# microsoft/MaskFlownet

Hardware: NVIDIA H100
Metric: image-pairs/sec (MaskFlownet-S forward, 1024x448) (higher is better)
Workload: dtype f32

## Files before the change

### include/maskflow_b200.h

```cpp
#ifndef MASKFLOW_B200_H_
#define MASKFLOW_B200_H_

#ifdef __cplusplus
extern "C" {
#endif

#define MFN_VERSION 100

#if defined(__GNUC__)
#define MFN_API __attribute__((visibility("default")))
#else
#define MFN_API
#endif

#define MFN_OK 0
#define MFN_ERR_INVALID_ARG (-1)
#define MFN_ERR_UNSUPPORTED (-2)
#define MFN_ERR_ALIGNMENT (-3)

#define MFN_CORR_AUTO 0
#define MFN_CORR_GENERIC 1
#define MFN_CORR_SIMT 2
#define MFN_CORR_MMA_BF16X3 3

#define MFN_BORDER_MXNET15 0
#define MFN_BORDER_ZERO_CORNER 1

MFN_API int mfn_version(void);
MFN_API const char* mfn_last_error(void);
MFN_API const char* mfn_last_kernel(void);
MFN_API unsigned long long mfn_launch_count(void);
MFN_API int mfn_set_tuning(const char* key, int value);

MFN_API int mfn_correlation_forward(const float* data1, const float* data2, float* out, int N, int C, int H,
                            int W, int pad_size, int kernel_size, int max_displacement, int stride1,
                            int stride2, int is_multiply, long long out_batch_stride,
                            float leaky_slope, int algo, void* stream);

MFN_API int mfn_correlation_backward(const float* grad_out, const float* out, const float* data1,
                             const float* data2, float* grad1, float* grad2, int N, int C, int H,
                             int W, int max_displacement, long long out_batch_stride,
                             float leaky_slope, void* stream);

MFN_API int mfn_deformable_conv_forward(const float* data, const float* offset, const float* weight,
                                const float* bias, float* out, int N, int C, int H, int W, int F,
                                int kernel_h, int kernel_w, int stride_h, int stride_w, int dilate_h,
                                int dilate_w, int pad_h, int pad_w, int num_group,
                                int num_deformable_group, int border_mode, void* stream);

MFN_API int mfn_deformable_conv_backward(const float* grad_out, const float* data, const float* offset,
                                 const float* weight, float* grad_data, float* grad_offset,
                                 float* grad_weight, float* grad_bias, int N, int C, int H, int W,
                                 int F, int border_mode, void* stream);

MFN_API int mfn_warp_mask_forward(const float* x, const float* flow_coarse, const float* mask_coarse,
                          const float* weight, const float* bias, const float* tradeoff, float* out,
                          float* flow_up_out, float* mask_up_out, float* conv_out, int N, int C,
                          int H, int W, int F, int upsample_factor, float flow_scale,
                          float level_stride, float leaky_slope, int border_mode, void* stream);

MFN_API int mfn_warp_mask_forward_tc(const float* x, const float* flow_coarse, const float* mask_coarse,
                                     const void* packed_weight, const float* bias, const float* tradeoff, float* out,
                                     float* flow_up_out, float* mask_up_out, float* conv_out, int N, int C, int H, int W,
                                     int F, int upsample_factor, float flow_scale, float level_stride, float leaky_slope,
                                     int border_mode, void* stream);

MFN_API long long mfn_warp_resample_workspace_bytes(int N, int F, int H, int W);
MFN_API int mfn_warp_mask_forward_resample(const float* x, const float* flow_coarse, const float* mask_coarse,
                                           const float* weight, const void* packed_weight, const float* bias,
                                           const float* tradeoff, void* workspace, float* out, float* flow_up_out,
                                           float* mask_up_out, int N, int C, int H, int W, int F, int upsample_factor,
                                           float flow_scale, float level_stride, float leaky_slope, int border_mode,
                                           void* stream);

MFN_API int mfn_warp_mask_backward(const float* grad_out, const float* out, const float* conv_out,
                           const float* x, const float* flow_up, const float* mask_up,
                           const float* weight, float* grad_x, float* grad_flow_up,
                           float* grad_mask_up, float* grad_weight, float* grad_bias,
                           float* grad_tradeoff, float* grad_conv_ws, int N, int C, int H, int W,
                           int F, float flow_scale, float level_stride, float leaky_slope,
                           int border_mode, void* stream);

MFN_API int mfn_upsample_forward(const float* in, float* out, int planes, int H, int W, int factor,
                         float scale, void* stream);
MFN_API int mfn_upsample_backward(const float* grad_out, float* grad_in, int planes, int H, int W, int factor,
                          float scale, void* stream);

MFN_API int mfn_grid_generator_warp_forward(const float* flow_xy, float* grid, int N, int H, int W,
                                    void* stream);
MFN_API int mfn_bilinear_sampler_forward(const float* data, const float* grid, float* out, int N, int C,
                                 int H, int W, int OH, int OW, void* stream);

MFN_API int mfn_grid_generator_warp_backward(const float* grad_grid, float* grad_flow, int N, int H, int W,
                                             void* stream);

MFN_API int mfn_bilinear_sampler_backward(const float* grad_out, const float* data, const float* grid,
                                          float* grad_data, float* grad_grid, int N, int C, int H, int W, int OH,
                                          int OW, void* stream);

MFN_API int mfn_image_warp_concat_forward(const float* im1, const float* im2, const float* flow_q,
                                  const float* mask_q, float* c30, float* c40, int N, int Ci, int H,
                                  int W, float flow_scale, void* stream);

MFN_API int mfn_image_warp_concat_backward(const float* grad_c40, const float* im2, const float* flow_q,
                                           const float* mask_q, float* grad_im2, float* grad_flow_up,
                                           float* grad_mask_up, int N, int Ci, int H, int W, float flow_scale,
                                           void* stream);

MFN_API long long mfn_conv3x3_packed_bytes(int Cin, int Cout);
MFN_API int mfn_conv3x3_pack_weights(const float* weight , void* packed, int Cin, int Cout,
                                     void* stream);
MFN_API int mfn_conv3x3_forward(const float* x, long long x_batch_stride, const void* packed_weight, const float* bias,
                                float* out, long long out_batch_stride, int N, int Cin, int H, int W, int Cout,
                                int dilation ,
                                float leaky_slope, void* stream);
#define MFN_CONV_OUT_NCHW 0
#define MFN_CONV_OUT_DEPTH_TO_SPACE2 1
#define MFN_CONV_OUT_LINEAR_PREFIX(k) ((k) << 8)
MFN_API int mfn_conv3x3_forward_ex(const float* x, long long x_batch_stride, const void* packed_weight, const float* bias,
                                   float* out, long long out_batch_stride, int N, int Cin, int H, int W, int Cout,
                                   int stride, int dilation, int out_mode, float leaky_slope, void* stream);
MFN_API long long mfn_conv3x3_workspace_bytes(int N, int Cin, int H, int W, int Cout, int stride, int dilation);
MFN_API int mfn_conv3x3_forward_ws(const float* x, long long x_batch_stride, const void* packed_weight, const float* bias,
                                   float* out, long long out_batch_stride, int N, int Cin, int H, int W, int Cout,
                                   int stride, int dilation, int out_mode, float leaky_slope, void* workspace,
                                   long long workspace_bytes, void* stream);

MFN_API int mfn_split_pack(const float* src, long long src_batch_stride, int N, int C, int H, int W, void* dst,
                           int dst_channels, int dst_c0, void* stream);
MFN_API int mfn_conv3x3_forward_split(const void* x, int x_channels, int x_c0, const void* packed_weight, const float* bias,
                                      float* out, long long out_batch_stride, void* out_split, int out_split_channels,
                                      int out_split_c0, int N, int Cin, int H, int W, int Cout, int dilation, int out_mode,
                                      float leaky_slope, void* workspace, long long workspace_bytes, void* stream);

MFN_API int mfn_preprocess_forward(const void* img1, const void* img2, int is_uint8, float* out1, float* out2,
                                   float* rgb_mean, int N, int C, int H, int W, int OH, int OW, void* stream);
MFN_API int mfn_postprocess_forward(const float* pred, float* out, int N, int channels, int Hq, int Wq, int H, int W,
                                    int flip_channels, int is_flow, void* stream);

MFN_API int mfn_flow_to_color(const float* flow_xy, unsigned char* rgb, float* rad_max, int N, int H, int W,
                              float max_radius, int bgr, void* stream);

MFN_API int mfn_warp_mask_backward_det(const float* grad_out, const float* out, const float* conv_out,
                                       const float* x, const float* flow_up, const float* mask_up,
                                       const float* weight, float* grad_x, float* grad_flow_up,
                                       float* grad_mask_up, float* grad_weight, float* grad_bias,
                                       float* grad_tradeoff, float* grad_conv_ws, int N, int C, int H, int W,
                                       int F, float flow_scale, float level_stride, float leaky_slope,
                                       int border_mode, void* det_ws, long long det_ws_bytes, void* stream);
MFN_API int mfn_deformable_conv_backward_det(const float* grad_out, const float* data, const float* offset,
                                             const float* weight, float* grad_data, float* grad_offset,
                                             float* grad_weight, float* grad_bias, int N, int C, int H, int W,
                                             int F, int border_mode, void* det_ws, long long det_ws_bytes,
                                             void* stream);
MFN_API int mfn_bilinear_sampler_backward_det(const float* grad_out, const float* data, const float* grid,
                                              float* grad_data, float* grad_grid, int N, int C, int H, int W,
                                              int OH, int OW, void* det_ws, long long det_ws_bytes, void* stream);
MFN_API int mfn_image_warp_concat_backward_det(const float* grad_c40, const float* im2, const float* flow_q,
                                               const float* mask_q, float* grad_im2, float* grad_flow_up,
                                               float* grad_mask_up, int N, int Ci, int H, int W, float flow_scale,
                                               void* det_ws, long long det_ws_bytes, void* stream);
MFN_API int mfn_preprocess_forward_det(const void* img1, const void* img2, int is_uint8, float* out1, float* out2,
                                       float* rgb_mean, int N, int C, int H, int W, int OH, int OW, void* det_ws,
                                       long long det_ws_bytes, void* stream);

MFN_API int mfn_geometry_augment_forward(const void* img1, const void* img2, int is_uint8, const float* flow, const void* mask,
                                         int mask_broadcast, const float* params, float* out_img1, float* out_img2,
                                         float* out_flow, float* out_mask, int N, int H, int W, int TH, int TW, void* stream);
MFN_API long long mfn_color_augment_workspace_bytes(int N);
MFN_API int mfn_color_augment_forward(const float* img1, const float* img2, const float* params, const float* noise1,
                                      const float* noise2, float noise_sigma, long long seed, float* out1, float* out2,
                                      void* workspace, long long workspace_bytes, int N, int H, int W, int has_gamma,
                                      void* stream);

MFN_API long long mfn_multiscale_epe_workspace_bytes(int N);
MFN_API int mfn_multiscale_epe_forward(const float* flow, const float* mask, const float* const* preds, const int* scales,
                                       const float* weights, int num_scales, float eps, float q, float* loss, float* mask_sum,
                                       void* workspace, long long workspace_bytes, int N, int H, int W, void* stream);
MFN_API int mfn_multiscale_epe_backward(const float* flow, const float* mask, const float* const* preds, const int* scales,
                                        const float* weights, int num_scales, float eps, float q, const float* grad_loss,
                                        const float* mask_sum, float* const* grad_preds, int N, int H, int W, void* stream);

#ifdef __cplusplus
}
#endif
#endif
```

### maskflownet_b200/_lib.py

```python
from __future__ import annotations

import ctypes
import os
import subprocess

_HERE = os.path.dirname(os.path.abspath(__file__))
SO_PATH = os.environ.get("MFN_LIB_PATH") or os.path.join(_HERE, "libmaskflow_b200.so")
_lib = None

_f = ctypes.c_void_p
_i = ctypes.c_int
_ll = ctypes.c_longlong
_fl = ctypes.c_float

SIGNATURES = {
    "mfn_correlation_forward": [_f, _f, _f, _i, _i, _i, _i, _i, _i, _i, _i, _i, _i, _ll, _fl, _i, _f],
    "mfn_correlation_backward": [_f, _f, _f, _f, _f, _f, _i, _i, _i, _i, _i, _ll, _fl, _f],
    "mfn_deformable_conv_forward": [_f, _f, _f, _f, _f] + [_i] * 16 + [_f],
    "mfn_deformable_conv_backward": [_f] * 8 + [_i] * 6 + [_f],
    "mfn_warp_mask_forward": [_f] * 10 + [_i] * 6 + [_fl, _fl, _fl, _i, _f],
    "mfn_warp_mask_forward_tc": [_f] * 10 + [_i] * 6 + [_fl, _fl, _fl, _i, _f],
    "mfn_warp_mask_forward_resample": [_f] * 11 + [_i] * 6 + [_fl, _fl, _fl, _i, _f],
    "mfn_warp_mask_backward": [_f] * 14 + [_i] * 5 + [_fl, _fl, _fl, _i, _f],
    "mfn_upsample_forward": [_f, _f, _i, _i, _i, _i, _fl, _f],
    "mfn_upsample_backward": [_f, _f, _i, _i, _i, _i, _fl, _f],
    "mfn_grid_generator_warp_forward": [_f, _f, _i, _i, _i, _f],
    "mfn_bilinear_sampler_forward": [_f, _f, _f, _i, _i, _i, _i, _i, _i, _f],
    "mfn_image_warp_concat_forward": [_f] * 6 + [_i] * 4 + [_fl, _f],
    "mfn_grid_generator_warp_backward": [_f, _f, _i, _i, _i, _f],
    "mfn_bilinear_sampler_backward": [_f] * 5 + [_i] * 6 + [_f],
    "mfn_image_warp_concat_backward": [_f] * 7 + [_i] * 4 + [_fl, _f],
    "mfn_preprocess_forward": [_f, _f, _i, _f, _f, _f, _i, _i, _i, _i, _i, _i, _f],
    "mfn_postprocess_forward": [_f, _f, _i, _i, _i, _i, _i, _i, _i, _i, _f],
    "mfn_flow_to_color": [_f, _f, _f, _i, _i, _i, _fl, _i, _f],
    "mfn_warp_mask_backward_det": [_f] * 14 + [_i] * 5 + [_fl, _fl, _fl, _i, _f, _ll, _f],
    "mfn_deformable_conv_backward_det": [_f] * 8 + [_i] * 6 + [_f, _ll, _f],
    "mfn_bilinear_sampler_backward_det": [_f] * 5 + [_i] * 6 + [_f, _ll, _f],
    "mfn_image_warp_concat_backward_det": [_f] * 7 + [_i] * 4 + [_fl, _f, _ll, _f],
    "mfn_preprocess_forward_det": [_f, _f, _i, _f, _f, _f, _i, _i, _i, _i, _i, _i, _f, _ll, _f],
    "mfn_geometry_augment_forward": [_f, _f, _i, _f, _f, _i, _f, _f, _f, _f, _f, _i, _i, _i, _i, _i, _f],
    "mfn_color_augment_forward": [_f, _f, _f, _f, _f, _fl, _ll, _f, _f, _f, _ll, _i, _i, _i, _i, _f],
    "mfn_multiscale_epe_forward": [_f, _f, _f, _f, _f, _i, _fl, _fl, _f, _f, _f, _ll, _i, _i, _i, _f],
    "mfn_multiscale_epe_backward": [_f, _f, _f, _f, _f, _i, _fl, _fl, _f, _f, _f, _i, _i, _i, _f],
    "mfn_set_tuning": [ctypes.c_char_p, _i],
    "mfn_conv3x3_pack_weights": [_f, _f, _i, _i, _f],
    "mfn_conv3x3_forward": [_f, _ll, _f, _f, _f, _ll, _i, _i, _i, _i, _i, _i, _fl, _f],
    "mfn_conv3x3_forward_ex": [_f, _ll, _f, _f, _f, _ll, _i, _i, _i, _i, _i, _i, _i, _i, _fl, _f],
    "mfn_conv3x3_forward_ws": [_f, _ll, _f, _f, _f, _ll, _i, _i, _i, _i, _i, _i, _i, _i, _fl, _f, _ll, _f],
    "mfn_conv3x3_forward_split": [_f, _i, _i, _f, _f, _f, _ll, _f, _i, _i] + [_i] * 7 + [_fl, _f, _ll, _f],
    "mfn_split_pack": [_f, _ll, _i, _i, _i, _i, _f, _i, _i, _f],
}


class MaskflowError(RuntimeError):
    pass


def build(verbose: bool = False) -> str:
    cmd = ["make", "-C", os.path.join(_HERE, "csrc"), "-j8"]
    res = subprocess.run(cmd, capture_output=not verbose, text=True)
    if res.returncode != 0:
        raise MaskflowError("building libmaskflow_b200.so failed:\n" + (res.stdout or "") + (res.stderr or ""))
    return SO_PATH


def lib() -> ctypes.CDLL:
    global _lib
    if _lib is None:
        if not os.path.exists(SO_PATH):
            raise MaskflowError(
                f"{SO_PATH} is missing: run `python -c 'import __graft_entry__ as g; g.build()'` "
                "(or `make -C maskflownet_b200/csrc`).  There is no CPU / PyTorch fallback for the hot path.")
        L = ctypes.CDLL(SO_PATH)
        L.mfn_version.restype = ctypes.c_int
        L.mfn_last_error.restype = ctypes.c_char_p
        L.mfn_last_kernel.restype = ctypes.c_char_p
        L.mfn_launch_count.restype = ctypes.c_ulonglong
        L.mfn_conv3x3_packed_bytes.restype = ctypes.c_longlong
        L.mfn_conv3x3_packed_bytes.argtypes = [ctypes.c_int, ctypes.c_int]
        L.mfn_conv3x3_workspace_bytes.restype = ctypes.c_longlong
        L.mfn_conv3x3_workspace_bytes.argtypes = [ctypes.c_int] * 7
        L.mfn_color_augment_workspace_bytes.restype = ctypes.c_longlong
        L.mfn_color_augment_workspace_bytes.argtypes = [ctypes.c_int]
        L.mfn_multiscale_epe_workspace_bytes.restype = ctypes.c_longlong
        L.mfn_multiscale_epe_workspace_bytes.argtypes = [ctypes.c_int]
        L.mfn_warp_resample_workspace_bytes.restype = ctypes.c_longlong
        L.mfn_warp_resample_workspace_bytes.argtypes = [ctypes.c_int] * 4
        for name, argtypes in SIGNATURES.items():
            fn = getattr(L, name)
            fn.argtypes = argtypes
            fn.restype = ctypes.c_int
        _lib = L
        for item in filter(None, os.environ.get("MFN_TUNING", "").split(",")):
            key, _, val = item.partition("=")
            if key.strip() in ("corr_dbg", "conv_dbg"):
                raise MaskflowError(f"MFN_TUNING: {key.strip()} is a profiling switch (results invalid); set it from a tool, "
                                    "not the environment")
            if L.mfn_set_tuning(key.strip().encode(), int(val)):
                raise MaskflowError(f"MFN_TUNING: {L.mfn_last_error().decode()}")
    return _lib


def last_error() -> str:
    return lib().mfn_last_error().decode()


def last_kernel() -> str:
    return lib().mfn_last_kernel().decode()


def launch_count() -> int:
    return int(lib().mfn_launch_count())


def call(name: str, *args) -> None:
    rc = getattr(lib(), name)(*args)
    if rc != 0:
        kind = "argument/support error" if rc < 0 else "CUDA error"
        raise MaskflowError(f"{name} failed ({kind} {rc}): {last_error()}")


def set_tuning(key: str, value: int) -> None:
    call("mfn_set_tuning", key.encode(), int(value))
```

### maskflownet_b200/csrc/api.cu

```cuda
#include <atomic>
#include <cstdarg>
#include <cstdio>
#include <cstring>

#include "common.cuh"

namespace mfn {

static thread_local char g_err[512] = "";
static thread_local const char* g_kernel = "";
static std::atomic<unsigned long long> g_launches{0};

int fail(int code, const char* fmt, ...) {
  va_list ap;
  va_start(ap, fmt);
  vsnprintf(g_err, sizeof(g_err), fmt, ap);
  va_end(ap);
  return code;
}

void note_kernel(const char* name) { g_kernel = name; }

Tuning& tuning() {
  static Tuning t;
  return t;
}

int check_launch(const char* kernel_name) {
  const cudaError_t e = cudaGetLastError();
  if (e != cudaSuccess) return fail((int)e, "%s: launch failed: %s", kernel_name, cudaGetErrorString(e));
  g_kernel = kernel_name;
  g_launches.fetch_add(1, std::memory_order_relaxed);
  g_err[0] = '\0';
  return MFN_OK;
}

}

extern "C" int mfn_version(void) { return MFN_VERSION; }
extern "C" const char* mfn_last_error(void) { return mfn::g_err; }
extern "C" const char* mfn_last_kernel(void) { return mfn::g_kernel; }
extern "C" unsigned long long mfn_launch_count(void) { return mfn::g_launches.load(std::memory_order_relaxed); }

extern "C" int mfn_set_tuning(const char* key, int value) {
  if (!key) return mfn::fail(MFN_ERR_INVALID_ARG, "mfn_set_tuning: null key");
  if (!strcmp(key, "corr_grid_cap")) mfn::tuning().corr_grid_cap = value;
  else if (!strcmp(key, "corr_disable_ring")) mfn::tuning().corr_disable_ring = value;
  else if (!strcmp(key, "warp_lin")) mfn::tuning().warp_lin = value;
  else if (!strcmp(key, "corr_rb")) mfn::tuning().corr_rb = value;
  else if (!strcmp(key, "warp_lin_fch")) mfn::tuning().warp_lin_fch = value;
  else if (!strcmp(key, "conv_as")) mfn::tuning().conv_as = value;
  else if (!strcmp(key, "conv_splitk")) mfn::tuning().conv_splitk = value;
  else if (!strcmp(key, "corr_rb_twb")) mfn::tuning().corr_rb_twb = value;
  else if (!strcmp(key, "corr_rb_rows")) mfn::tuning().corr_rb_rows = value;
  else if (!strcmp(key, "corr_tma")) mfn::tuning().corr_tma = value;
  else if (!strcmp(key, "corr_ts_lo")) mfn::tuning().corr_ts_lo = value;
  else if (!strcmp(key, "corr_ts_hi")) mfn::tuning().corr_ts_hi = value;
  else if (!strcmp(key, "corr_dbg")) mfn::tuning().corr_dbg = value;
  else if (!strcmp(key, "conv_dbg")) mfn::tuning().conv_dbg = value;
  else if (!strcmp(key, "corr_ring_th")) mfn::tuning().corr_ring_th = value;
  else if (!strcmp(key, "conv_wgmma")) mfn::tuning().conv_wgmma = value;
  else if (!strcmp(key, "conv_grid_cap")) mfn::tuning().conv_grid_cap = value;
  else if (!strcmp(key, "conv_wgmma_min_w")) mfn::tuning().conv_wgmma_min_w = value;
  else return mfn::fail(MFN_ERR_INVALID_ARG, "mfn_set_tuning: unknown key '%s'", key);
  return MFN_OK;
}
```

### maskflownet_b200/csrc/common.cuh

```cuda
#pragma once
#include <cuda_runtime.h>
#include <stdint.h>

#include "../../include/maskflow_b200.h"
#include "device_caps.h"
#include "sampling.cuh"

namespace mfn {

int fail(int code, const char* fmt, ...);
int check_launch(const char* kernel_name);
void note_kernel(const char* name);

struct Tuning {
  int corr_grid_cap = 0;
  int corr_disable_ring = 0;
  int conv_wgmma = 1;
  int conv_grid_cap = 0;
  int conv_wgmma_min_w = 1;
  int corr_ring_th = 8;
  int corr_rb = 1;
  int warp_lin_fch = 0;
  int conv_as = 0;
  int conv_splitk = 1;
  int corr_rb_twb = 0;
  int corr_rb_rows = 0;
  int corr_tma = 1;
  int warp_lin = 1;
  int corr_ts_lo = 0, corr_ts_hi = 0;
  int corr_dbg = 0;
  int conv_dbg = 0;
};
Tuning& tuning();

static inline cudaStream_t as_stream(void* s) { return reinterpret_cast<cudaStream_t>(s); }

#define MFN_REQUIRE(cond, code, ...)                   \
  do {                                                 \
    if (!(cond)) return ::mfn::fail(code, __VA_ARGS__); \
  } while (0)

static inline bool aligned(const void* p, size_t a) { return (reinterpret_cast<uintptr_t>(p) % a) == 0; }

static inline unsigned grid_for(long long total, int threads) {
  long long b = (total + threads - 1) / threads;
  const long long cap = (long long)kNumSMs * 16;
  return (unsigned)(b < cap ? (b > 0 ? b : 1) : cap);
}


struct SmemOptIn {
  int bytes[64] = {};
};
template <typename K>
static inline cudaError_t ensure_dyn_smem(K kernel, int bytes, SmemOptIn& st) {
  int dev = 0;
  if (cudaGetDevice(&dev) != cudaSuccess) dev = -1;
  if (dev >= 0 && dev < 64 && st.bytes[dev] >= bytes) return cudaSuccess;
  const cudaError_t e = cudaFuncSetAttribute(kernel, cudaFuncAttributeMaxDynamicSharedMemorySize, bytes);
  if (e == cudaSuccess && dev >= 0 && dev < 64) st.bytes[dev] = bytes;
  return e;
}

long long warp_lin_workspace_bytes(int N, int F, int H, int W);
int launch_warp_lin(const float* x, const float* flow_c, const float* mask_c, const float* weight, const void* packed_weight,
                    const float* bias, const float* tradeoff, void* workspace, float* out, float* fup, float* mup, int N,
                    int C, int H, int W, int F, int up, float fs, float ls, float slope, int border_mode, cudaStream_t st);

int launch_corr_rb(int md, const float* d1, const float* d2, float* out, int N, int C, int H, int W, long long obs,
                   float slope, cudaStream_t st);

int launch_corr_tma(int md, const float* d1, const float* d2, float* out, int N, int C, int H, int W, long long obs,
                    float slope, cudaStream_t st);

int det_launch_abs_max(const float* v, long long n, unsigned* bound, cudaStream_t st);
int det_launch_pixel_abs_sum_max(const float* g, int N, int F, long long HW, unsigned* bound, cudaStream_t st);
int det_launch_fixed_to_float(const unsigned long long* acc, float* out, long long n, const unsigned* bound, int nb,
                              int fanin_bits, cudaStream_t st);
int det_launch_ordered_sum(const float* part, int nparts, long long part_stride, long long elem_stride, float* out,
                           long long n, int accumulate, cudaStream_t st);
int det_check_workspace(const char* fn, const void* ws, long long bytes, long long need);

__device__ __forceinline__ float leaky(float v, float slope) { return v > 0.f ? v : v * slope; }


struct Tap {
  int h0, h1, w0, w1;
  float lh, lw;
  bool valid;
  bool c00, c01, c10, c11;
};

template <int BORDER>
__device__ __forceinline__ Tap make_tap(float h, float w, int H, int W) {
  Tap t;
  if (BORDER == MFN_BORDER_MXNET15) {
    t.valid = (h >= 0.f) && (w >= 0.f) && (h < (float)H) && (w < (float)W);
    int h0 = (int)floorf(h), w0 = (int)floorf(w);
    if (h0 >= H - 1) {
      h0 = H - 1;
      t.h1 = h0;
      t.lh = 0.f;
    } else {
      t.h1 = h0 + 1;
      t.lh = h - (float)h0;
    }
    if (w0 >= W - 1) {
      w0 = W - 1;
      t.w1 = w0;
      t.lw = 0.f;
    } else {
      t.w1 = w0 + 1;
      t.lw = w - (float)w0;
    }
    t.h0 = h0;
    t.w0 = w0;
    if (!t.valid) {
      t.h0 = t.h1 = t.w0 = t.w1 = 0;
      t.lh = t.lw = 0.f;
    }
    t.c00 = t.c01 = t.c10 = t.c11 = t.valid;
  } else {
    t.valid = (h > -1.f) && (w > -1.f) && (h < (float)H) && (w < (float)W);
    const int h0 = (int)floorf(h), w0 = (int)floorf(w);
    t.lh = h - (float)h0;
    t.lw = w - (float)w0;
    const bool hin0 = h0 >= 0, hin1 = h0 + 1 <= H - 1, win0 = w0 >= 0, win1 = w0 + 1 <= W - 1;
    t.c00 = t.valid && hin0 && win0;
    t.c01 = t.valid && hin0 && win1;
    t.c10 = t.valid && hin1 && win0;
    t.c11 = t.valid && hin1 && win1;
    t.h0 = max(min(h0, H - 1), 0);
    t.h1 = max(min(h0 + 1, H - 1), 0);
    t.w0 = max(min(w0, W - 1), 0);
    t.w1 = max(min(w0 + 1, W - 1), 0);
    if (!t.valid) t.lh = t.lw = 0.f;
  }
  return t;
}

__device__ __forceinline__ float tap_sample(const Tap& t, const float* __restrict__ plane, int W) {
  const float hh = 1.f - t.lh, hw = 1.f - t.lw;
  float v = 0.f;
  if (t.c00) v += hh * hw * __ldg(plane + (size_t)t.h0 * W + t.w0);
  if (t.c01) v += hh * t.lw * __ldg(plane + (size_t)t.h0 * W + t.w1);
  if (t.c10) v += t.lh * hw * __ldg(plane + (size_t)t.h1 * W + t.w0);
  if (t.c11) v += t.lh * t.lw * __ldg(plane + (size_t)t.h1 * W + t.w1);
  return v;
}

}
```

### maskflownet_b200/csrc/conv3x3.cu

```cuda
#include "mma_tiles.cuh"

namespace mfn {
__global__ void conv3x3_pack_kernel(const float* __restrict__ w, unsigned char* __restrict__ packed, int Cin, int Cout,
                                    int CoutP, int nChunks) {
  using namespace c3;
  const long long total = (long long)nChunks * 9 * CoutP * 16;
  for (long long i = (long long)blockIdx.x * blockDim.x + threadIdx.x; i < total; i += (long long)gridDim.x * blockDim.x) {
    const int j = (int)(i & 15);
    const int f = (int)((i >> 4) % CoutP);
    const int tap = (int)((i / (16LL * CoutP)) % 9);
    const int q = (int)(i / (16LL * CoutP * 9));
    const int c = 32 * q + 2 * j;
    float a = 0.f, b = 0.f;
    if (f < Cout) {
      if (c < Cin) a = w[((size_t)f * Cin + c) * 9 + tap];
      if (c + 1 < Cin) b = w[((size_t)f * Cin + c + 1) * 9 + tap];
    }
    uint32_t hi, lo;
    split_pair(a, b, hi, lo);
    unsigned char* tile = packed + ((size_t)q * 9 + tap) * (2 * CoutP * PXB);
    const int off = swz(f, j >> 2) + (j & 3) * 4;
    *reinterpret_cast<uint32_t*>(tile + off) = hi;
    *reinterpret_cast<uint32_t*>(tile + CoutP * PXB + off) = lo;
  }
}

template <int WC, int NTN, bool PT>
__global__ void __launch_bounds__(c3::NTHREADS, 1)
    conv3x3_mma_kernel(const float* __restrict__ x, long long x_bs, const unsigned char* __restrict__ wpack,
                       const float* __restrict__ bias, float* __restrict__ out, long long out_bs, int Cin, int H, int W,
                       int Cout, int CoutP, int nChunks, float slope, int tilesX, int tilesY, int dil, int lin_prefix) {
  using namespace c3;
  constexpr int WR = 8 / WC;
  constexpr int TROWS = PT ? WR : WR + 2;
  constexpr int HWP = PT ? TW : c3::HWP;
  constexpr int IN_LO = TROWS * HWP * PXB;
  constexpr int IN_STAGE = 2 * IN_LO;
  const int WT_LO = CoutP * PXB;
  const int WT_BYTES = 2 * WT_LO;

  extern __shared__ __align__(128) unsigned char smem[];
  unsigned char* in_s = smem;
  unsigned char* wt_s = smem + 2 * IN_STAGE;

  const int tid = threadIdx.x, warp = tid >> 5, lane = tid & 31;
  const int wr = warp / WC, wc = warp % WC;
  const int tile = blockIdx.x;
  const int tx = tile % tilesX, ty = (tile / tilesX) % tilesY, n = tile / (tilesX * tilesY);
  const int x0 = tx * TW, y0 = ty * WR;
  const size_t plane = (size_t)H * W;
  const float* xn = x + (size_t)n * x_bs;

  constexpr int U_MAIN = TROWS * 4;
  constexpr int U_HALO = PT ? 0 : ((TROWS + 3) / 4) * 4;
  constexpr int U_TOT = U_MAIN + U_HALO;
  constexpr int UPW = (U_TOT + 7) / 8;
  auto unit_geom = [&](int u, int& row, int& chunk, int& pidx, int& xx, bool& act) {
    act = u < U_TOT;
    if (u < U_MAIN) {
      row = u >> 2;
      chunk = u & 3;
      pidx = PT ? lane : HX + lane;
      xx = x0 + lane;
    } else {
      const int k = u - U_MAIN;
      row = 4 * (k >> 2) + (lane >> 3);
      chunk = k & 3;
      const int px8 = lane & 7;
      pidx = px8 < 4 ? px8 : TW + px8;
      xx = px8 < 4 ? x0 - HX + px8 : x0 + TW + (px8 - 4);
      act = act && row < TROWS;
    }
  };
  auto load_tile = [&](int q, float (&e)[UPW][8]) {
    int sy = -1, sx = 0;
    if (PT) {
      const int tap = q % 9;
      sy = (tap / 3 - 1) * dil;
      sx = (tap % 3 - 1) * dil;
      q /= 9;
    }
#pragma unroll
    for (int k = 0; k < UPW; ++k) {
      int row, chunk, pidx, xx;
      bool act;
      unit_geom(warp * UPW + k, row, chunk, pidx, xx, act);
      xx += sx;
      const int yy = y0 + sy + row;
      const bool ok = act && yy >= 0 && yy < H && xx >= 0 && xx < W;
      const int c0 = 32 * q + 8 * chunk;
      const float* p = xn + (size_t)c0 * plane + (size_t)yy * W + xx;
#pragma unroll
      for (int c = 0; c < 8; ++c) {
        e[k][c] = (ok && c0 + c < Cin) ? __ldg(p) : 0.f;
        p += plane;
      }
    }
  };
  auto store_tile = [&](int stage, const float (&e)[UPW][8]) {
#pragma unroll
    for (int k = 0; k < UPW; ++k) {
      int row, chunk, pidx, xx;
      bool act;
      unit_geom(warp * UPW + k, row, chunk, pidx, xx, act);
      if (!act) continue;
      uint4 hi, lo;
      split_pair(e[k][0], e[k][1], hi.x, lo.x);
      split_pair(e[k][2], e[k][3], hi.y, lo.y);
      split_pair(e[k][4], e[k][5], hi.z, lo.z);
      split_pair(e[k][6], e[k][7], hi.w, lo.w);
      unsigned char* dst = in_s + stage * IN_STAGE + row * (HWP * PXB) + swz(pidx, chunk);
      *reinterpret_cast<uint4*>(dst) = hi;
      *reinterpret_cast<uint4*>(dst + IN_LO) = lo;
    }
  };
  auto load_weights = [&](int it, int stage) {
    const unsigned char* src = wpack + (size_t)it * WT_BYTES;
    const uint32_t dst = smem_u32(wt_s + stage * WT_BYTES);
    for (int o = tid * 16; o < WT_BYTES; o += NTHREADS * 16) cp_async16(dst + o, src + o);
  };

  const int g = lane >> 2, j = lane & 3;
  const int l8 = lane & 7, mi = lane >> 3;
  const int swB = (l8 >> 1) & 3;
  uint32_t offB[2];
#pragma unroll
  for (int kk = 0; kk < 2; ++kk) offB[kk] = (uint32_t)((8 * (mi >> 1) + l8) * PXB + (((2 * kk + (mi & 1)) ^ swB) << 4));
  const int fbase = wc * NTN * 8;

  float acc[2][NTN][4];
#pragma unroll
  for (int mt = 0; mt < 2; ++mt)
#pragma unroll
    for (int nt = 0; nt < NTN; ++nt)
#pragma unroll
      for (int i = 0; i < 4; ++i) acc[mt][nt][i] = 0.f;

  const int nIter = nChunks * 9;
  {
    float e[UPW][8];
    load_tile(0, e);
    store_tile(0, e);
  }
  load_weights(0, 0);
  cp_async_commit();
  if (nIter > 1) load_weights(1, 1);
  cp_async_commit();

  const uint32_t in_u32 = smem_u32(in_s), wt_u32 = smem_u32(wt_s);
  float pe[UPW][8];
  for (int it = 0; it < nIter; ++it) {
    const int q = it / 9, tap = it - 9 * q;
    const int ky = tap / 3, kx = tap - 3 * ky;
    cp_async_wait<1>();
    __syncthreads();
    if (it + 2 < nIter) load_weights(it + 2, (it + 2) % WSTAGES);
    cp_async_commit();
    if (PT) {
      if (it + 1 < nIter) load_tile(it + 1, pe);
    } else {
      if (tap == 0 && q + 1 < nChunks) load_tile(q + 1, pe);
      if (tap == 8 && q + 1 < nChunks) store_tile((q + 1) & 1, pe);
    }

    const uint32_t wst = wt_u32 + (uint32_t)((it % WSTAGES) * WT_BYTES);
    const uint32_t ist = PT ? in_u32 + (uint32_t)((it & 1) * IN_STAGE + wr * (HWP * PXB))
                            : in_u32 + (uint32_t)((q & 1) * IN_STAGE + (wr + ky) * (HWP * PXB));
    const bool half_chunk = 32 * q + 16 >= Cin;
#pragma unroll
    for (int kk = 0; kk < 2; ++kk) {
      if (kk == 1 && half_chunk) break;
      uint32_t ah[2][4], al[2][4];
#pragma unroll
      for (int mt = 0; mt < 2; ++mt) {
        const int p = (PT ? 0 : HX - 1 + kx) + 16 * mt + 8 * (mi & 1) + l8;
        const uint32_t a = ist + (uint32_t)(p * PXB + (((2 * kk + (mi >> 1)) ^ ((p >> 1) & 3)) << 4));
        ldsm_x4(a, ah[mt]);
        ldsm_x4(a + IN_LO, al[mt]);
      }
#pragma unroll
      for (int nt = 0; nt < NTN; nt += 2) {
        uint32_t bh[4], bl[4];
        const uint32_t b = wst + (uint32_t)((fbase + 8 * nt) * PXB) + offB[kk];
        ldsm_x4(b, bh);
        ldsm_x4(b + WT_LO, bl);
#pragma unroll
        for (int mt = 0; mt < 2; ++mt) {
          mma_bf16(acc[mt][nt], ah[mt], bl[0], bl[1]);
          mma_bf16(acc[mt][nt], al[mt], bh[0], bh[1]);
          mma_bf16(acc[mt][nt], ah[mt], bh[0], bh[1]);
          if (nt + 1 < NTN) {
            mma_bf16(acc[mt][nt + 1], ah[mt], bl[2], bl[3]);
            mma_bf16(acc[mt][nt + 1], al[mt], bh[2], bh[3]);
            mma_bf16(acc[mt][nt + 1], ah[mt], bh[2], bh[3]);
          }
        }
      }
    }
    if (PT && it + 1 < nIter) store_tile((it + 1) & 1, pe);
  }

  const int y = y0 + wr;
  if (y >= H) return;
  float* on = out + (size_t)n * out_bs + (size_t)y * W;
#pragma unroll
  for (int nt = 0; nt < NTN; ++nt) {
#pragma unroll
    for (int i = 0; i < 4; ++i) {
      const int f = fbase + 8 * nt + 2 * j + (i & 1);
      if (f >= Cout) continue;
      const float b = bias ? __ldg(bias + f) : 0.f;
#pragma unroll
      for (int mt = 0; mt < 2; ++mt) {
        const int xx = x0 + 16 * mt + g + 8 * (i >> 1);
        if (xx < W) on[(size_t)f * plane + xx] = leaky(acc[mt][nt][i] + b, f < lin_prefix ? 1.f : slope);
      }
    }
  }
}

template <int WC, int NTN, bool PT>
static int launch_conv_impl(const float* x, long long x_bs, const unsigned char* wpack, const float* bias, float* out,
                            long long out_bs, int N, int Cin, int H, int W, int Cout, int dil, float slope, int lin_prefix,
                            cudaStream_t st) {
  using namespace c3;
  constexpr int WR = 8 / WC;
  const int CoutP = cout_pad(Cout);
  const int nChunks = (Cin + 31) / 32;
  const int tilesX = (W + TW - 1) / TW, tilesY = (H + WR - 1) / WR;
  const int in_stage = PT ? 2 * WR * TW * PXB : 2 * (WR + 2) * HWP * PXB;
  const int smem = 2 * in_stage + WSTAGES * 2 * CoutP * PXB;
  static SmemOptIn opt;
  {
    const cudaError_t e = ensure_dyn_smem(conv3x3_mma_kernel<WC, NTN, PT>, smem, opt);
    if (e != cudaSuccess) return fail((int)e, "cudaFuncSetAttribute(conv3x3_mma_kernel): %s", cudaGetErrorString(e));
  }
  const unsigned grid = (unsigned)((long long)N * tilesX * tilesY);
  conv3x3_mma_kernel<WC, NTN, PT><<<grid, NTHREADS, smem, st>>>(x, x_bs, wpack, bias, out, out_bs, Cin, H, W, Cout,
                                                               CoutP, nChunks, slope, tilesX, tilesY, dil, lin_prefix);
  return check_launch(PT ? "conv3x3_mma_kernel<per-tap tiles>" : "conv3x3_mma_kernel<halo tile>");
}

template <int WC, int NTN>
static int launch_conv(const float* x, long long x_bs, const unsigned char* wpack, const float* bias, float* out,
                       long long out_bs, int N, int Cin, int H, int W, int Cout, int dil, float slope, int lin_prefix,
                       cudaStream_t st) {
  return dil == 1 ? launch_conv_impl<WC, NTN, false>(x, x_bs, wpack, bias, out, out_bs, N, Cin, H, W, Cout, 1, slope, lin_prefix, st)
                  : launch_conv_impl<WC, NTN, true>(x, x_bs, wpack, bias, out, out_bs, N, Cin, H, W, Cout, dil, slope, lin_prefix, st);
}

long long conv3x3_sync_packed_bytes(int Cin, int Cout) {
  if (Cout > 128) return 0;
  return (long long)((Cin + 31) / 32) * 9 * 2 * c3::cout_pad(Cout) * c3::PXB;
}

}

extern "C" long long mfn_conv3x3_packed_bytes(int Cin, int Cout) {
  if (Cin <= 0 || Cout <= 0) return 0;
  return mfn::conv3x3_sync_packed_bytes(Cin, Cout) + mfn::conv3x3_wgmma_packed_bytes(Cin, Cout);
}

extern "C" int mfn_conv3x3_pack_weights(const float* weight, void* packed, int Cin, int Cout, void* stream) {
  using namespace mfn;
  MFN_REQUIRE(weight && packed, MFN_ERR_INVALID_ARG, "mfn_conv3x3_pack_weights: null pointer");
  MFN_REQUIRE(Cin > 0 && Cout > 0, MFN_ERR_INVALID_ARG, "mfn_conv3x3_pack_weights: non-positive extent");
  MFN_REQUIRE(aligned(packed, 16), MFN_ERR_ALIGNMENT, "mfn_conv3x3_pack_weights: packed buffer must be 16-byte aligned");
  MFN_REQUIRE(Cout <= 256, MFN_ERR_UNSUPPORTED, "mfn_conv3x3_pack_weights: at most 256 output channels (got %d)", Cout);
  if (Cout <= 128) {
    const int CoutP = c3::cout_pad(Cout), nChunks = (Cin + 31) / 32;
    const long long total = (long long)nChunks * 9 * CoutP * 16;
    long long blocks = (total + 255) / 256;
    if (blocks > 4096) blocks = 4096;
    conv3x3_pack_kernel<<<(unsigned)blocks, 256, 0, as_stream(stream)>>>(weight, static_cast<unsigned char*>(packed), Cin,
                                                                         Cout, CoutP, nChunks);
    const int rc = check_launch("conv3x3_pack_kernel");
    if (rc) return rc;
  }
  return conv3x3_wgmma_pack(weight, static_cast<unsigned char*>(packed) + conv3x3_sync_packed_bytes(Cin, Cout), Cin, Cout,
                           as_stream(stream));
}

extern "C" int mfn_conv3x3_forward(const float* x, long long x_batch_stride, const void* packed_weight,
                                   const float* bias, float* out, long long out_batch_stride, int N, int Cin, int H,
                                   int W, int Cout, int dilation, float leaky_slope, void* stream) {
  return mfn_conv3x3_forward_ex(x, x_batch_stride, packed_weight, bias, out, out_batch_stride, N, Cin, H, W, Cout, 1,
                                dilation, MFN_CONV_OUT_NCHW, leaky_slope, stream);
}

extern "C" int mfn_conv3x3_forward_ex(const float* x, long long x_batch_stride, const void* packed_weight,
                                      const float* bias, float* out, long long out_batch_stride, int N, int Cin, int H,
                                      int W, int Cout, int stride, int dilation, int out_mode, float leaky_slope,
                                      void* stream) {
  return mfn_conv3x3_forward_ws(x, x_batch_stride, packed_weight, bias, out, out_batch_stride, N, Cin, H, W, Cout, stride,
                                dilation, out_mode, leaky_slope, nullptr, 0, stream);
}

extern "C" long long mfn_conv3x3_workspace_bytes(int N, int Cin, int H, int W, int Cout, int stride, int dilation) {
  using namespace mfn;
  if (N <= 0 || Cin <= 0 || H <= 0 || W <= 0 || Cout <= 0 || Cout > 256 || dilation < 1 ||
      !(stride == 1 || (stride == 2 && dilation == 1)))
    return 0;
  if (!(tuning().conv_wgmma && W >= tuning().conv_wgmma_min_w) && Cout <= 128 && stride == 1) return 0;
  return conv3x3_wgmma_workspace_bytes(N, Cin, H, W, Cout, stride, dilation);
}

extern "C" int mfn_conv3x3_forward_ws(const float* x, long long x_batch_stride, const void* packed_weight,
                                      const float* bias, float* out, long long out_batch_stride, int N, int Cin, int H,
                                      int W, int Cout, int stride, int dilation, int out_mode, float leaky_slope,
                                      void* workspace, long long workspace_bytes, void* stream) {
  using namespace mfn;
  MFN_REQUIRE(workspace_bytes >= 0 && (workspace || workspace_bytes == 0) && aligned(workspace, 16), MFN_ERR_INVALID_ARG,
              "mfn_conv3x3_forward_ws: workspace must be 16-byte aligned (or null with 0 bytes)");
  MFN_REQUIRE(x && packed_weight && out, MFN_ERR_INVALID_ARG, "mfn_conv3x3_forward: null pointer");
  MFN_REQUIRE(N > 0 && Cin > 0 && H > 0 && W > 0 && Cout > 0, MFN_ERR_INVALID_ARG,
              "mfn_conv3x3_forward: non-positive extent");
  MFN_REQUIRE(Cout <= 256, MFN_ERR_UNSUPPORTED, "mfn_conv3x3_forward: at most 256 output channels (got %d)", Cout);
  MFN_REQUIRE(dilation >= 1, MFN_ERR_INVALID_ARG, "mfn_conv3x3_forward: dilation must be >= 1");
  MFN_REQUIRE(stride == 1 || (stride == 2 && dilation == 1), MFN_ERR_UNSUPPORTED,
              "mfn_conv3x3_forward: stride must be 1, or 2 with dilation 1 (got stride %d, dilation %d)", stride, dilation);
  MFN_REQUIRE(aligned(packed_weight, 16), MFN_ERR_ALIGNMENT, "mfn_conv3x3_forward: packed weights must be 16-byte aligned");
  const int lin_prefix = out_mode >> 8, mode = out_mode & 0xff;
  MFN_REQUIRE(mode == MFN_CONV_OUT_NCHW || (mode == MFN_CONV_OUT_DEPTH_TO_SPACE2 && stride == 1 && Cout % 4 == 0),
              MFN_ERR_INVALID_ARG, "mfn_conv3x3_forward: depth-to-space output needs stride 1 and Cout %% 4 == 0");
  MFN_REQUIRE(lin_prefix >= 0 && lin_prefix <= Cout && (lin_prefix == 0 || mode == MFN_CONV_OUT_NCHW), MFN_ERR_INVALID_ARG,
              "mfn_conv3x3_forward: linear prefix (out_mode >> 8 = %d) needs NCHW output and <= Cout", lin_prefix);
  const int OH = (H - 1) / stride + 1, OW = (W - 1) / stride + 1;
  const long long xbs = x_batch_stride ? x_batch_stride : (long long)Cin * H * W;
  const long long obs = out_batch_stride ? out_batch_stride : (long long)Cout * OH * OW;
  MFN_REQUIRE(xbs >= (long long)Cin * H * W && obs >= (long long)Cout * OH * OW, MFN_ERR_INVALID_ARG,
              "mfn_conv3x3_forward: batch stride smaller than the tensor");
  const unsigned char* wp = static_cast<const unsigned char*>(packed_weight);
  cudaStream_t st = as_stream(stream);
  const bool sync_ok = Cout <= 128 && stride == 1 && mode == MFN_CONV_OUT_NCHW;
  if ((tuning().conv_wgmma && W >= tuning().conv_wgmma_min_w) || !sync_ok) {
    const int rc = conv3x3_wgmma_launch(x, xbs, wp + conv3x3_sync_packed_bytes(Cin, Cout), bias, out, obs, N, Cin, H, W,
                                       Cout, stride, dilation, out_mode, leaky_slope, st, 0, static_cast<float*>(workspace),
                                       workspace_bytes);
    if (rc != -1) return rc;
    MFN_REQUIRE(sync_ok, MFN_ERR_UNSUPPORTED, "mfn_conv3x3_forward: shape fits neither kernel (Cout=%d stride=%d dilation=%d)",
                Cout, stride, dilation);
  }
  const int nt = (Cout + 7) / 8;
  if (nt <= 4) return launch_conv<1, 4>(x, xbs, wp, bias, out, obs, N, Cin, H, W, Cout, dilation, leaky_slope, lin_prefix, st);
  if (nt <= 8) return launch_conv<1, 8>(x, xbs, wp, bias, out, obs, N, Cin, H, W, Cout, dilation, leaky_slope, lin_prefix, st);
  if (nt <= 12) return launch_conv<2, 6>(x, xbs, wp, bias, out, obs, N, Cin, H, W, Cout, dilation, leaky_slope, lin_prefix, st);
  return launch_conv<2, 8>(x, xbs, wp, bias, out, obs, N, Cin, H, W, Cout, dilation, leaky_slope, lin_prefix, st);
}

extern "C" int mfn_conv3x3_forward_split(const void* x, int x_channels, int x_c0, const void* packed_weight,
                                         const float* bias, float* out, long long out_batch_stride, void* out_split,
                                         int out_split_channels, int out_split_c0, int N, int Cin, int H, int W, int Cout,
                                         int dilation, int out_mode, float leaky_slope, void* workspace,
                                         long long workspace_bytes, void* stream) {
  using namespace mfn;
  MFN_REQUIRE(workspace_bytes >= 0 && (workspace || workspace_bytes == 0) && aligned(workspace, 16), MFN_ERR_INVALID_ARG,
              "mfn_conv3x3_forward_split: workspace must be 16-byte aligned (or null with 0 bytes)");
  const int lin_prefix = out_mode >> 8, mode = out_mode & 0xff;
  MFN_REQUIRE(x && packed_weight && (out || (out_split && lin_prefix == 0)), MFN_ERR_INVALID_ARG,
              "mfn_conv3x3_forward_split: null pointer");
  MFN_REQUIRE(N > 0 && Cin > 0 && H > 0 && W > 0 && Cout > 0 && Cout <= 256 && dilation >= 1, MFN_ERR_INVALID_ARG,
              "mfn_conv3x3_forward_split: bad extent, Cout (<= 256) or dilation");
  MFN_REQUIRE(x_c0 >= 0 && x_c0 % 16 == 0 && x_c0 + Cin <= x_channels &&
                  ((x_c0 + Cin) % 16 == 0 || x_c0 + Cin == x_channels),
              MFN_ERR_INVALID_ARG,
              "mfn_conv3x3_forward_split: input slice [%d, %d) of the %d channels must start at a multiple of 16 and end "
              "at one or at the last channel", x_c0, x_c0 + Cin, x_channels);
  MFN_REQUIRE(aligned(packed_weight, 16) && aligned(x, 16), MFN_ERR_ALIGNMENT,
              "mfn_conv3x3_forward_split: packed weights and split input must be 16-byte aligned");
  MFN_REQUIRE(lin_prefix >= 0 && lin_prefix <= Cout && (lin_prefix == 0 || mode == MFN_CONV_OUT_NCHW), MFN_ERR_INVALID_ARG,
              "mfn_conv3x3_forward_split: linear prefix needs NCHW / split output and <= Cout");
  MFN_REQUIRE(mode == MFN_CONV_OUT_NCHW || (mode == MFN_CONV_OUT_DEPTH_TO_SPACE2 && Cout % 4 == 0 && !out_split),
              MFN_ERR_INVALID_ARG, "mfn_conv3x3_forward_split: depth-to-space output needs Cout %% 4 == 0 and fp32 output");
  const int Fo = out_split ? lin_prefix : (mode ? Cout / 4 : Cout), OS = mode ? 4 : 1;
  const long long obs = out_batch_stride ? out_batch_stride : (long long)Fo * H * W * OS;
  MFN_REQUIRE(obs >= (long long)Fo * H * W * OS, MFN_ERR_INVALID_ARG, "mfn_conv3x3_forward_split: batch stride too small");
  SplitIO sio;
  sio.in = x;
  sio.in_C = x_channels;
  sio.in_c0 = x_c0;
  sio.out = out_split;
  sio.out_C = out_split_channels;
  sio.out_c0 = out_split_c0;
  const unsigned char* wp = static_cast<const unsigned char*>(packed_weight);
  const int rc = conv3x3_wgmma_launch(nullptr, 0, wp + conv3x3_sync_packed_bytes(Cin, Cout), bias, out, obs, N, Cin, H, W,
                                      Cout, 1, dilation, out_mode, leaky_slope, as_stream(stream), 0,
                                      static_cast<float*>(workspace), workspace_bytes, sio);
  MFN_REQUIRE(rc != -1, MFN_ERR_UNSUPPORTED,
              "mfn_conv3x3_forward_split: unsupported (odd dilation >= 2, split output slice not 16-channel aligned "
              "after an even linear prefix, or too large)");
  return rc;
}
```

### maskflownet_b200/csrc/conv3x3_wgmma.cu

```cuda
#include <cstring>

#include "mma_tiles.cuh"
#include "split_act.cuh"

namespace mfn {
namespace um {
constexpr int MT = 128;
constexpr int R = 2;
constexpr int NTHREADS = 384;
constexpr int NCONS = 8;
constexpr int NPROD = 3;
constexpr int MAX_AS = 4, MAX_WS = 24;
constexpr int BATCH = 6;
constexpr int BAR_BYTES = 1024;

__host__ __device__ inline int n_slots(int stride, int dil) { return stride == 2 ? 2 * R + 1 : (dil >= R ? 3 * R : R + 2 * dil); }
__host__ __device__ inline int row_pitch(int stride, int dil) { return stride == 2 ? 2 * MT + 1 : MT + 2 * dil; }
__host__ __device__ inline int slot_of(int r, int ky, int stride, int dil) {
  return stride == 2 ? 2 * r + ky : (dil >= R ? ky * R + r : r + ky * dil);
}
__host__ __device__ inline int tap_xoff(int kx, int stride, int dil) {
  return stride == 2 ? (kx == 1 ? 0 : (kx == 0 ? MT : MT + 1)) : kx * dil;
}
__host__ __device__ inline int band_map(int v, int n) { return v < n ? v : (v == n + 2 ? 0 : (v == n + 5 ? n - 1 : -1)); }
__host__ __device__ inline int cout_pad(int cout) { return cout <= 128 ? (cout + 15) / 16 * 16 : 256; }
__host__ __device__ inline bool fold_hi_lo(int CoutP) { return CoutP <= 64; }
__host__ __device__ inline int taps_per_stage(int CoutP) { return CoutP <= 32 ? 9 : (CoutP <= 64 ? 3 : 1); }

__device__ __forceinline__ uint64_t desc_hi(uint32_t lbo_bytes, uint32_t sbo_bytes) {
  return ((uint64_t)((lbo_bytes >> 4) & 0x3FFFu) << 16) | ((uint64_t)((sbo_bytes >> 4) & 0x3FFFu) << 32);
}
__device__ __forceinline__ void wgmma_fence() { asm volatile("wgmma.fence.sync.aligned;" ::: "memory"); }
__device__ __forceinline__ void wgmma_commit() { asm volatile("wgmma.commit_group.sync.aligned;" ::: "memory"); }
template <int N>
__device__ __forceinline__ void wgmma_wait() { asm volatile("wgmma.wait_group.sync.aligned %0;" ::"n"(N) : "memory"); }
template <int S>
__device__ __forceinline__ void fence_acc(float (&d)[S]) {
#pragma unroll
  for (int i = 0; i < S; ++i) asm volatile("" : "+f"(d[i])::"memory");
}
template <int S>
__device__ __forceinline__ void wgmma_n16(float (&d)[S], uint64_t a, uint64_t b, uint32_t scale_d) {
  static_assert(S >= 8, "accumulator too small");
  asm volatile(
      "{\n\t.reg .pred p;\n\tsetp.ne.b32 p, %10, 0;\n\t"
      "wgmma.mma_async.sync.aligned.m64n16k16.f32.bf16.bf16 {%0, %1, %2, %3, %4, %5, %6, %7}, %8, %9, p, 1, 1, 0, 0;\n\t}"
      : "+f"(d[0]), "+f"(d[1]), "+f"(d[2]), "+f"(d[3]), "+f"(d[4]), "+f"(d[5]), "+f"(d[6]), "+f"(d[7])
      : "l"(a), "l"(b), "r"(scale_d));
}
template <int S>
__device__ __forceinline__ void wgmma_n32(float (&d)[S], uint64_t a, uint64_t b, uint32_t scale_d) {
  static_assert(S >= 16, "accumulator too small");
  asm volatile(
      "{\n\t.reg .pred p;\n\tsetp.ne.b32 p, %18, 0;\n\t"
      "wgmma.mma_async.sync.aligned.m64n32k16.f32.bf16.bf16 {%0, %1, %2, %3, %4, %5, %6, %7, %8, %9, %10, %11, %12, %13, %14, %15}, %16, %17, p, 1, 1, 0, 0;\n\t}"
      : "+f"(d[0]), "+f"(d[1]), "+f"(d[2]), "+f"(d[3]), "+f"(d[4]), "+f"(d[5]), "+f"(d[6]), "+f"(d[7]), "+f"(d[8]), "+f"(d[9]), "+f"(d[10]), "+f"(d[11]), "+f"(d[12]), "+f"(d[13]), "+f"(d[14]), "+f"(d[15])
      : "l"(a), "l"(b), "r"(scale_d));
}
template <int S>
__device__ __forceinline__ void wgmma_n48(float (&d)[S], uint64_t a, uint64_t b, uint32_t scale_d) {
  static_assert(S >= 24, "accumulator too small");
  asm volatile(
      "{\n\t.reg .pred p;\n\tsetp.ne.b32 p, %26, 0;\n\t"
      "wgmma.mma_async.sync.aligned.m64n48k16.f32.bf16.bf16 {%0, %1, %2, %3, %4, %5, %6, %7, %8, %9, %10, %11, %12, %13, %14, %15, %16, %17, %18, %19, %20, %21, %22, %23}, %24, %25, p, 1, 1, 0, 0;\n\t}"
      : "+f"(d[0]), "+f"(d[1]), "+f"(d[2]), "+f"(d[3]), "+f"(d[4]), "+f"(d[5]), "+f"(d[6]), "+f"(d[7]), "+f"(d[8]), "+f"(d[9]), "+f"(d[10]), "+f"(d[11]), "+f"(d[12]), "+f"(d[13]), "+f"(d[14]), "+f"(d[15]), "+f"(d[16]), "+f"(d[17]), "+f"(d[18]), "+f"(d[19]), "+f"(d[20]), "+f"(d[21]), "+f"(d[22]), "+f"(d[23])
      : "l"(a), "l"(b), "r"(scale_d));
}
template <int S>
__device__ __forceinline__ void wgmma_n64(float (&d)[S], uint64_t a, uint64_t b, uint32_t scale_d) {
  static_assert(S >= 32, "accumulator too small");
  asm volatile(
      "{\n\t.reg .pred p;\n\tsetp.ne.b32 p, %34, 0;\n\t"
      "wgmma.mma_async.sync.aligned.m64n64k16.f32.bf16.bf16 {%0, %1, %2, %3, %4, %5, %6, %7, %8, %9, %10, %11, %12, %13, %14, %15, %16, %17, %18, %19, %20, %21, %22, %23, %24, %25, %26, %27, %28, %29, %30, %31}, %32, %33, p, 1, 1, 0, 0;\n\t}"
      : "+f"(d[0]), "+f"(d[1]), "+f"(d[2]), "+f"(d[3]), "+f"(d[4]), "+f"(d[5]), "+f"(d[6]), "+f"(d[7]), "+f"(d[8]), "+f"(d[9]), "+f"(d[10]), "+f"(d[11]), "+f"(d[12]), "+f"(d[13]), "+f"(d[14]), "+f"(d[15]), "+f"(d[16]), "+f"(d[17]), "+f"(d[18]), "+f"(d[19]), "+f"(d[20]), "+f"(d[21]), "+f"(d[22]), "+f"(d[23]), "+f"(d[24]), "+f"(d[25]), "+f"(d[26]), "+f"(d[27]), "+f"(d[28]), "+f"(d[29]), "+f"(d[30]), "+f"(d[31])
      : "l"(a), "l"(b), "r"(scale_d));
}
template <int S>
__device__ __forceinline__ void wgmma_n80(float (&d)[S], uint64_t a, uint64_t b, uint32_t scale_d) {
  static_assert(S >= 40, "accumulator too small");
  asm volatile(
      "{\n\t.reg .pred p;\n\tsetp.ne.b32 p, %42, 0;\n\t"
      "wgmma.mma_async.sync.aligned.m64n80k16.f32.bf16.bf16 {%0, %1, %2, %3, %4, %5, %6, %7, %8, %9, %10, %11, %12, %13, %14, %15, %16, %17, %18, %19, %20, %21, %22, %23, %24, %25, %26, %27, %28, %29, %30, %31, %32, %33, %34, %35, %36, %37, %38, %39}, %40, %41, p, 1, 1, 0, 0;\n\t}"
      : "+f"(d[0]), "+f"(d[1]), "+f"(d[2]), "+f"(d[3]), "+f"(d[4]), "+f"(d[5]), "+f"(d[6]), "+f"(d[7]), "+f"(d[8]), "+f"(d[9]), "+f"(d[10]), "+f"(d[11]), "+f"(d[12]), "+f"(d[13]), "+f"(d[14]), "+f"(d[15]), "+f"(d[16]), "+f"(d[17]), "+f"(d[18]), "+f"(d[19]), "+f"(d[20]), "+f"(d[21]), "+f"(d[22]), "+f"(d[23]), "+f"(d[24]), "+f"(d[25]), "+f"(d[26]), "+f"(d[27]), "+f"(d[28]), "+f"(d[29]), "+f"(d[30]), "+f"(d[31]), "+f"(d[32]), "+f"(d[33]), "+f"(d[34]), "+f"(d[35]), "+f"(d[36]), "+f"(d[37]), "+f"(d[38]), "+f"(d[39])
      : "l"(a), "l"(b), "r"(scale_d));
}
template <int S>
__device__ __forceinline__ void wgmma_n96(float (&d)[S], uint64_t a, uint64_t b, uint32_t scale_d) {
  static_assert(S >= 48, "accumulator too small");
  asm volatile(
      "{\n\t.reg .pred p;\n\tsetp.ne.b32 p, %50, 0;\n\t"
      "wgmma.mma_async.sync.aligned.m64n96k16.f32.bf16.bf16 {%0, %1, %2, %3, %4, %5, %6, %7, %8, %9, %10, %11, %12, %13, %14, %15, %16, %17, %18, %19, %20, %21, %22, %23, %24, %25, %26, %27, %28, %29, %30, %31, %32, %33, %34, %35, %36, %37, %38, %39, %40, %41, %42, %43, %44, %45, %46, %47}, %48, %49, p, 1, 1, 0, 0;\n\t}"
      : "+f"(d[0]), "+f"(d[1]), "+f"(d[2]), "+f"(d[3]), "+f"(d[4]), "+f"(d[5]), "+f"(d[6]), "+f"(d[7]), "+f"(d[8]), "+f"(d[9]), "+f"(d[10]), "+f"(d[11]), "+f"(d[12]), "+f"(d[13]), "+f"(d[14]), "+f"(d[15]), "+f"(d[16]), "+f"(d[17]), "+f"(d[18]), "+f"(d[19]), "+f"(d[20]), "+f"(d[21]), "+f"(d[22]), "+f"(d[23]), "+f"(d[24]), "+f"(d[25]), "+f"(d[26]), "+f"(d[27]), "+f"(d[28]), "+f"(d[29]), "+f"(d[30]), "+f"(d[31]), "+f"(d[32]), "+f"(d[33]), "+f"(d[34]), "+f"(d[35]), "+f"(d[36]), "+f"(d[37]), "+f"(d[38]), "+f"(d[39]), "+f"(d[40]), "+f"(d[41]), "+f"(d[42]), "+f"(d[43]), "+f"(d[44]), "+f"(d[45]), "+f"(d[46]), "+f"(d[47])
      : "l"(a), "l"(b), "r"(scale_d));
}
template <int S>
__device__ __forceinline__ void wgmma_n112(float (&d)[S], uint64_t a, uint64_t b, uint32_t scale_d) {
  static_assert(S >= 56, "accumulator too small");
  asm volatile(
      "{\n\t.reg .pred p;\n\tsetp.ne.b32 p, %58, 0;\n\t"
      "wgmma.mma_async.sync.aligned.m64n112k16.f32.bf16.bf16 {%0, %1, %2, %3, %4, %5, %6, %7, %8, %9, %10, %11, %12, %13, %14, %15, %16, %17, %18, %19, %20, %21, %22, %23, %24, %25, %26, %27, %28, %29, %30, %31, %32, %33, %34, %35, %36, %37, %38, %39, %40, %41, %42, %43, %44, %45, %46, %47, %48, %49, %50, %51, %52, %53, %54, %55}, %56, %57, p, 1, 1, 0, 0;\n\t}"
      : "+f"(d[0]), "+f"(d[1]), "+f"(d[2]), "+f"(d[3]), "+f"(d[4]), "+f"(d[5]), "+f"(d[6]), "+f"(d[7]), "+f"(d[8]), "+f"(d[9]), "+f"(d[10]), "+f"(d[11]), "+f"(d[12]), "+f"(d[13]), "+f"(d[14]), "+f"(d[15]), "+f"(d[16]), "+f"(d[17]), "+f"(d[18]), "+f"(d[19]), "+f"(d[20]), "+f"(d[21]), "+f"(d[22]), "+f"(d[23]), "+f"(d[24]), "+f"(d[25]), "+f"(d[26]), "+f"(d[27]), "+f"(d[28]), "+f"(d[29]), "+f"(d[30]), "+f"(d[31]), "+f"(d[32]), "+f"(d[33]), "+f"(d[34]), "+f"(d[35]), "+f"(d[36]), "+f"(d[37]), "+f"(d[38]), "+f"(d[39]), "+f"(d[40]), "+f"(d[41]), "+f"(d[42]), "+f"(d[43]), "+f"(d[44]), "+f"(d[45]), "+f"(d[46]), "+f"(d[47]), "+f"(d[48]), "+f"(d[49]), "+f"(d[50]), "+f"(d[51]), "+f"(d[52]), "+f"(d[53]), "+f"(d[54]), "+f"(d[55])
      : "l"(a), "l"(b), "r"(scale_d));
}
template <int S>
__device__ __forceinline__ void wgmma_n128(float (&d)[S], uint64_t a, uint64_t b, uint32_t scale_d) {
  static_assert(S >= 64, "accumulator too small");
  asm volatile(
      "{\n\t.reg .pred p;\n\tsetp.ne.b32 p, %66, 0;\n\t"
      "wgmma.mma_async.sync.aligned.m64n128k16.f32.bf16.bf16 {%0, %1, %2, %3, %4, %5, %6, %7, %8, %9, %10, %11, %12, %13, %14, %15, %16, %17, %18, %19, %20, %21, %22, %23, %24, %25, %26, %27, %28, %29, %30, %31, %32, %33, %34, %35, %36, %37, %38, %39, %40, %41, %42, %43, %44, %45, %46, %47, %48, %49, %50, %51, %52, %53, %54, %55, %56, %57, %58, %59, %60, %61, %62, %63}, %64, %65, p, 1, 1, 0, 0;\n\t}"
      : "+f"(d[0]), "+f"(d[1]), "+f"(d[2]), "+f"(d[3]), "+f"(d[4]), "+f"(d[5]), "+f"(d[6]), "+f"(d[7]), "+f"(d[8]), "+f"(d[9]), "+f"(d[10]), "+f"(d[11]), "+f"(d[12]), "+f"(d[13]), "+f"(d[14]), "+f"(d[15]), "+f"(d[16]), "+f"(d[17]), "+f"(d[18]), "+f"(d[19]), "+f"(d[20]), "+f"(d[21]), "+f"(d[22]), "+f"(d[23]), "+f"(d[24]), "+f"(d[25]), "+f"(d[26]), "+f"(d[27]), "+f"(d[28]), "+f"(d[29]), "+f"(d[30]), "+f"(d[31]), "+f"(d[32]), "+f"(d[33]), "+f"(d[34]), "+f"(d[35]), "+f"(d[36]), "+f"(d[37]), "+f"(d[38]), "+f"(d[39]), "+f"(d[40]), "+f"(d[41]), "+f"(d[42]), "+f"(d[43]), "+f"(d[44]), "+f"(d[45]), "+f"(d[46]), "+f"(d[47]), "+f"(d[48]), "+f"(d[49]), "+f"(d[50]), "+f"(d[51]), "+f"(d[52]), "+f"(d[53]), "+f"(d[54]), "+f"(d[55]), "+f"(d[56]), "+f"(d[57]), "+f"(d[58]), "+f"(d[59]), "+f"(d[60]), "+f"(d[61]), "+f"(d[62]), "+f"(d[63])
      : "l"(a), "l"(b), "r"(scale_d));
}
template <int N, int S>
__device__ __forceinline__ void wgmma_bf16(float (&d)[S], uint64_t a, uint64_t b, uint32_t scale_d) {
  if constexpr (N == 16) wgmma_n16(d, a, b, scale_d);
  else if constexpr (N == 32) wgmma_n32(d, a, b, scale_d);
  else if constexpr (N == 48) wgmma_n48(d, a, b, scale_d);
  else if constexpr (N == 64) wgmma_n64(d, a, b, scale_d);
  else if constexpr (N == 80) wgmma_n80(d, a, b, scale_d);
  else if constexpr (N == 96) wgmma_n96(d, a, b, scale_d);
  else if constexpr (N == 112) wgmma_n112(d, a, b, scale_d);
  else wgmma_n128(d, a, b, scale_d);
}

struct SplitK {
  int k, from, n_lo, y_lo, rh;
  long long part_stride;
  float* ws;
  uint32_t magic_tp, magic_tx;
  int as_wide;
  int ns;
  int stg;
};
__device__ __forceinline__ void decode_tile(int tile, int tilesX, int tilesY, const SplitK& sk, int& tx, int& ty, int& n) {
  if (sk.magic_tp) {
    n = (int)__umulhi((uint32_t)tile, sk.magic_tp);
    const int rem = tile - n * tilesX * tilesY;
    ty = sk.magic_tx ? (int)__umulhi((uint32_t)rem, sk.magic_tx) : rem;
    tx = rem - ty * tilesX;
  } else {
    tx = tile % tilesX;
    ty = (tile / tilesX) % tilesY;
    n = tile / (tilesX * tilesY);
  }
}
struct SplitDev {
  int in, in_g0, in_Cg;
  unsigned char* out;
  int out_Cg, out_c0;
};
struct Work {
  int tile, part, cb, ce, nh;
};
__device__ __forceinline__ Work decode_work(int w, const SplitK& sk, int nChunks) {
  Work r;
  r.nh = 0;
  if (sk.ns == 2) {
    r.nh = w & 1;
    w >>= 1;
  }
  if (sk.k <= 1 || w < sk.from) {
    r.tile = w; r.part = -1; r.cb = 0; r.ce = nChunks;
  } else {
    const int u = w - sk.from, t = u / sk.k;
    r.tile = sk.from + t;
    r.part = u - t * sk.k;
    r.cb = r.part * nChunks / sk.k;
    r.ce = (r.part + 1) * nChunks / sk.k;
  }
  return r;
}

struct SmemMap {
  int a_lo, a_stage, w_tile, w_stage, w_off, bar_off, stg_off, total, AS, WS;
};
constexpr int STG_CH = 32, SPITCH = MT + 4;
constexpr int STG_BYTES = R * STG_CH * SPITCH * 4;
__host__ __device__ inline SmemMap smem_map(int E, int CoutP, int as_wide = 3, int stg = 0) {
  SmemMap m;
  m.a_lo = 2 * E * 16;
  m.a_stage = 2 * m.a_lo;
  m.w_tile = 64 * CoutP;
  const int budget = 227 * 1024 - BAR_BYTES - stg;
  m.w_stage = taps_per_stage(CoutP) * m.w_tile;
  if (taps_per_stage(CoutP) > 1)
    m.AS = (4 * m.a_stage + 4 * m.w_stage <= budget) ? 4 : ((3 * m.a_stage + 3 * m.w_stage <= budget) ? 3 : 2);
  else
    m.AS = (as_wide >= 3 && 3 * m.a_stage + 8 * m.w_stage <= budget) ? 3 : 2;
  int ws = (budget - m.AS * m.a_stage) / m.w_stage;
  m.WS = ws > MAX_WS ? MAX_WS : ws;
  m.w_off = m.AS * m.a_stage;
  m.bar_off = m.w_off + m.WS * m.w_stage;
  m.stg_off = m.bar_off + BAR_BYTES;
  m.total = m.stg_off + stg;
  return m;
}
}

__global__ void conv3x3_pack_wgmma_kernel(const float* __restrict__ w, unsigned char* __restrict__ packed, int Cin, int Cout,
                                          int CoutP, int nChunks16) {
  const long long total = (long long)nChunks16 * 9 * CoutP * 8;
  for (long long i = (long long)blockIdx.x * blockDim.x + threadIdx.x; i < total; i += (long long)gridDim.x * blockDim.x) {
    const int j = (int)(i & 7);
    const int f = (int)((i >> 3) % CoutP);
    const int tap = (int)((i / (8LL * CoutP)) % 9);
    const int c = (int)(i / (8LL * CoutP * 9));
    const int ch = 16 * c + 2 * j;
    float a = 0.f, b = 0.f;
    if (f < Cout) {
      if (ch < Cin) a = w[((size_t)f * Cin + ch) * 9 + tap];
      if (ch + 1 < Cin) b = w[((size_t)f * Cin + ch + 1) * 9 + tap];
    }
    uint32_t hi, lo;
    split_pair(a, b, hi, lo);
    const int wt = 64 * CoutP;
    unsigned char* tile = packed + ((size_t)c * 9 + tap) * wt;
    if (um::fold_hi_lo(CoutP)) {
      const int off = (j >> 2) * (2 * CoutP * 16) + f * 16 + (j & 3) * 4;
      *reinterpret_cast<uint32_t*>(tile + off) = hi;
      *reinterpret_cast<uint32_t*>(tile + CoutP * 16 + off) = lo;
    } else {
      const int off = (j >> 2) * (CoutP * 16) + f * 16 + (j & 3) * 4;
      *reinterpret_cast<uint32_t*>(tile + off) = hi;
      *reinterpret_cast<uint32_t*>(tile + wt / 2 + off) = lo;
    }
  }
}

template <int NW, bool FOLD, int TPS>
__global__ void __launch_bounds__(um::NTHREADS, 1)
    conv3x3_wgmma_kernel(const float* __restrict__ x, long long x_bs, const unsigned char* __restrict__ wpack,
                         const float* __restrict__ bias_arg, float* __restrict__ out_base, long long out_bs, int Cin, int H, int W,
                         int OH, int OW, int Cout, int CoutP, int nChunks, float slope_arg, int tilesX, int tilesY, int numWork,
                         int stride, int dil, int out_mode_arg, int ext, um::SplitK sk, um::SplitDev xs,
                         const __grid_constant__ CUtensorMap tmx, int dbg) {
  using namespace um;
  constexpr int NCOL = FOLD ? NW / 2 : NW;
  const int out_mode_k = out_mode_arg & 0xff, lin_prefix_k = out_mode_arg >> 8;
  extern __shared__ __align__(128) unsigned char smem[];
  const int nslots = n_slots(stride, dil), PW = row_pitch(stride, dil), E = nslots * PW;
  const SmemMap sm = smem_map(E, CoutP, sk.as_wide, sk.stg);
  const int AS = sm.AS, WS = sm.WS;
  const uint32_t s_base = smem_u32(smem);
  const uint32_t bar0 = s_base + sm.bar_off;
  const uint32_t a_full = bar0, a_empty = bar0 + 8 * MAX_AS, w_full = bar0 + 16 * MAX_AS, w_empty = w_full + 8 * MAX_WS;

  const int tid = threadIdx.x, lane = tid & 31;
  const int warp = __shfl_sync(0xffffffffu, tid >> 5, 0);
  const size_t plane = (size_t)H * W;

  if (tid == 0) {
    for (int i = 0; i < AS; ++i) {
      mbar_init(a_full + 8 * i, xs.in ? 1 : NPROD);
      mbar_init(a_empty + 8 * i, NCONS);
    }
    for (int i = 0; i < WS; ++i) {
      mbar_init(w_full + 8 * i, 1);
      mbar_init(w_empty + 8 * i, NCONS);
    }
    asm volatile("fence.mbarrier_init.release.cluster;" ::: "memory");
  }
  __syncthreads();

  if (warp < 8) {
    const int r = warp >> 2, wq = warp & 3;
    const uint32_t a_lbo = (uint32_t)E * 16u, b_lbo = (uint32_t)(FOLD ? 2 * CoutP : CoutP) * 16u;
    uint32_t a_off[9];
#pragma unroll
    for (int tap = 0; tap < 9; ++tap)
      a_off[tap] = (uint32_t)(slot_of(r, tap / 3, stride, dil) * PW + tap_xoff(tap % 3, stride, dil));
    const uint64_t dh_a = desc_hi(a_lbo, 128u), dh_b = desc_hi(b_lbo, 128u);
    uint32_t as = 0, aph = 0, ws = 0, wph = 0;
    const uint32_t a_lo16 = (uint32_t)sm.a_lo >> 4, a_stage16 = (uint32_t)sm.a_stage >> 4, s_base16 = s_base >> 4;
    const uint32_t w_base16 = (s_base + (uint32_t)sm.w_off) >> 4, w_tile16 = (uint32_t)sm.w_tile >> 4, w_half16 = w_tile16 >> 1;
    const uint32_t w_stage16 = (uint32_t)sm.w_stage >> 4;
    int rel_w = -1, rel_a = -1;
    auto release = [&]() {
      if (lane == 0) {
        if (rel_w >= 0) mbar_arrive(w_empty + 8 * rel_w);
        if (rel_a >= 0) mbar_arrive(a_empty + 8 * rel_a);
      }
      rel_w = rel_a = -1;
    };
    float acc[2][NW / 2];
    for (int work = blockIdx.x; work < numWork; work += gridDim.x) {
      const Work wk = decode_work(work, sk, nChunks);
      const int cb = wk.cb, ce = wk.ce;
      const uint32_t b_nh16 = (uint32_t)(wk.nh * NCOL);
      fence_acc(acc[0]);
      fence_acc(acc[1]);
      if (dbg & 8) {
        for (int c = cb; c < ce; ++c) {
          mbar_wait(a_full + 8 * as, aph);
          for (int tap = 0; tap < 9; ++tap) {
            if (tap % TPS == 0) mbar_wait(w_full + 8 * ws, wph);
            release();
            if (tap % TPS == TPS - 1) {
              rel_w = (int)ws;
              if (++ws == (uint32_t)WS) { ws = 0; wph ^= 1; }
            }
            if (tap == 8) rel_a = (int)as;
          }
          if (++as == (uint32_t)AS) { as = 0; aph ^= 1; }
        }
      }
      for (int c = (dbg & 8) ? ce : cb; c < ce; ++c) {
        mbar_wait(a_full + 8 * as, aph);
        const uint32_t a_st16 = s_base16 + as * a_stage16;
#pragma unroll
        for (int tap = 0; tap < 9; ++tap) {
          if (tap % TPS == 0) mbar_wait(w_full + 8 * ws, wph);
          const uint32_t w16 = w_base16 + ws * w_stage16 + (uint32_t)(tap % TPS) * w_tile16 + b_nh16;
          const uint64_t b_hi = dh_b | (uint64_t)w16, b_lo = dh_b | (uint64_t)(w16 + w_half16);
          const uint32_t sc = (tap == 0 && c == cb) ? 0u : 1u;
          wgmma_fence();
#pragma unroll
          for (int mh = 0; mh < 2; ++mh) {
            const uint32_t a16 = a_st16 + a_off[tap] + (uint32_t)(64 * mh);
            const uint64_t a_hi = dh_a | (uint64_t)a16, a_lo = dh_a | (uint64_t)(a16 + a_lo16);
            if constexpr (FOLD) {
              wgmma_bf16<NW>(acc[mh], a_hi, b_hi, sc);
              wgmma_bf16<NW / 2>(acc[mh], a_lo, b_hi, 1u);
            } else {
              wgmma_bf16<NW>(acc[mh], a_hi, b_lo, sc);
              wgmma_bf16<NW>(acc[mh], a_lo, b_hi, 1u);
              wgmma_bf16<NW>(acc[mh], a_hi, b_hi, 1u);
            }
          }
          wgmma_commit();
          wgmma_wait<1>();
          release();
          if (tap % TPS == TPS - 1) {
            rel_w = (int)ws;
            if (++ws == (uint32_t)WS) { ws = 0; wph ^= 1; }
          }
          if (tap == 8) rel_a = (int)as;
        }
        if (++as == (uint32_t)AS) { as = 0; aph ^= 1; }
      }
      wgmma_wait<0>();
      fence_acc(acc[0]);
      fence_acc(acc[1]);
      release();

      int tx, ty, n;
      decode_tile(wk.tile, tilesX, tilesY, sk, tx, ty, n);
      const bool partial = wk.part >= 0;
      const float* const bias = partial ? nullptr : bias_arg;
      const float slope = partial ? 1.f : slope_arg;
      const int out_mode = partial ? 0 : out_mode_k, lin_prefix = partial ? 0 : lin_prefix_k;
      const size_t oplane0 = partial ? (size_t)sk.rh * OW : (size_t)OH * OW;
      float* const out = partial ? sk.ws + (size_t)wk.part * (size_t)sk.part_stride + (size_t)(n - sk.n_lo) * Cout * oplane0 -
                                       (size_t)sk.y_lo * OW
                                 : out_base + (size_t)n * out_bs;
      const int y = ty * R + r;
      const int F = Cout >> 2;
      const size_t oplane2 = (size_t)(2 * OH) * (2 * OW);
      if (y < OH && !(dbg & 4) && sk.stg && !partial) {
        constexpr int SCH = NCOL % STG_CH == 0 ? STG_CH : 16;
        float* const stg = reinterpret_cast<float*>(smem + sm.stg_off) + r * STG_CH * SPITCH;
        const int t = wq * 32 + lane;
        const int x0 = tx * MT;
        const uint32_t seg = (uint32_t)((OW - x0 < MT ? OW - x0 : MT) * 4);
        if (xs.out != nullptr) {
          unsigned char* const sst = reinterpret_cast<unsigned char*>(stg);
#pragma unroll
          for (int pc = 0; pc < NCOL / SCH; ++pc) {
            if (t < SCH / 4) bulk_wait_read();
            named_bar_sync(1 + r, 128);
#pragma unroll
            for (int jj = 0; jj < SCH / 8; ++jj) {
              const int j = pc * (SCH / 8) + jj;
              const int f = wk.nh * NCOL + 8 * j + 2 * (lane & 3);
              const float b0 = (bias != nullptr && f < Cout) ? __ldg(bias + f) : 0.f;
              const float b1 = (bias != nullptr && f + 1 < Cout) ? __ldg(bias + f + 1) : 0.f;
              unsigned char* const row = sst + (2 * jj * MT + 16 * wq + (lane >> 2)) * 16 + (lane & 3) * 4;
#pragma unroll
              for (int mh = 0; mh < 2; ++mh)
#pragma unroll
                for (int h = 0; h < 2; ++h) {
                  const int i = 4 * j + 2 * h;
                  float v0 = acc[mh][i], v1 = acc[mh][i + 1];
                  if constexpr (FOLD) {
                    v0 += acc[mh][i + NW / 4];
                    v1 += acc[mh][i + 1 + NW / 4];
                  }
                  uint32_t hi, lo;
                  split_pair(leaky(v0 + b0, slope), leaky(v1 + b1, slope), hi, lo);
                  unsigned char* const e = row + (64 * mh + 8 * h) * 16;
                  *reinterpret_cast<uint32_t*>(e) = hi;
                  *reinterpret_cast<uint32_t*>(e + MT * 16) = lo;
                }
            }
            asm volatile("fence.proxy.async.shared::cta;" ::: "memory");
            named_bar_sync(1 + r, 128);
            const int f = wk.nh * NCOL + pc * SCH + 8 * (t >> 1);
            if (t < SCH / 4 && f < Cout) {
              const long long dst = sa::entry(n, t & 1, (xs.out_c0 + f) >> 3, (long long)y * OW + x0, xs.out_Cg, oplane0);
              bulk_s2g(xs.out + dst, smem_u32(sst + t * MT * 16), seg * 4);
              bulk_commit();
            }
          }
        } else
#pragma unroll
        for (int pc = 0; pc < NCOL / SCH; ++pc) {
          if (t < SCH) bulk_wait_read();
          named_bar_sync(1 + r, 128);
#pragma unroll
          for (int jj = 0; jj < SCH / 8; ++jj) {
            const int j = pc * (SCH / 8) + jj;
#pragma unroll
            for (int e = 0; e < 2; ++e) {
              const int f = wk.nh * NCOL + 8 * j + 2 * (lane & 3) + e;
              const float b = (bias != nullptr && f < Cout) ? __ldg(bias + f) : 0.f;
              const float sl = f < lin_prefix ? 1.f : slope;
              float* const row = stg + (8 * jj + 2 * (lane & 3) + e) * SPITCH + 16 * wq + (lane >> 2);
#pragma unroll
              for (int mh = 0; mh < 2; ++mh)
#pragma unroll
                for (int h = 0; h < 2; ++h) {
                  const int i = 4 * j + 2 * h + e;
                  float v = acc[mh][i];
                  if constexpr (FOLD) v += acc[mh][i + NW / 4];
                  row[64 * mh + 8 * h] = leaky(v + b, sl);
                }
            }
          }
          asm volatile("fence.proxy.async.shared::cta;" ::: "memory");
          named_bar_sync(1 + r, 128);
          const int f = wk.nh * NCOL + pc * SCH + t;
          if (t < SCH && f < Cout) {
            bulk_s2g(out + (size_t)f * oplane0 + (size_t)y * OW + x0, smem_u32(stg + t * SPITCH), seg);
            bulk_commit();
          }
        }
      } else if (y < OH && !(dbg & 4)) {
#pragma unroll
        for (int mh = 0; mh < 2; ++mh) {
#pragma unroll
          for (int h = 0; h < 2; ++h) {
            const int xx = tx * MT + 64 * mh + 16 * wq + (lane >> 2) + 8 * h;
            if (xx >= OW) continue;
#pragma unroll
            for (int j = 0; j < NCOL / 8; ++j) {
#pragma unroll
              for (int e = 0; e < 2; ++e) {
                const int i = 4 * j + 2 * h + e;
                float v = acc[mh][i];
                if constexpr (FOLD) v += acc[mh][i + NW / 4];
                const int f = wk.nh * NCOL + 8 * j + 2 * (lane & 3) + e;
                if (f >= Cout) continue;
                if (xs.out != nullptr && !partial && f >= lin_prefix) {
                  if (e == 0) {
                    const float b0 = bias != nullptr ? __ldg(bias + f) : 0.f, b1 = bias != nullptr ? __ldg(bias + f + 1) : 0.f;
                    float v1 = acc[mh][i + 1];
                    if constexpr (FOLD) v1 += acc[mh][i + 1 + NW / 4];
                    sa::put_pair(xs.out, xs.out_Cg, oplane0, n, xs.out_c0 + f - lin_prefix, (size_t)y * OW + xx,
                                 leaky(v + b0, slope), leaky(v1 + b1, slope));
                  }
                } else if (out_mode == 0) {
                  const float t = v + (bias != nullptr ? __ldg(bias + f) : 0.f);
                  out[(size_t)f * oplane0 + (size_t)y * OW + xx] = leaky(t, f < lin_prefix ? 1.f : slope);
                } else {
                  const int ph = f / F, ff = f - ph * F;
                  const float t = v + (bias != nullptr ? __ldg(bias + ff) : 0.f);
                  out[(size_t)ff * oplane2 + (size_t)(2 * y + (ph >> 1)) * (2 * OW) + 2 * xx + (ph & 1)] = leaky(t, slope);
                }
              }
            }
          }
        }
      }
    }
    bulk_wait_all();
  } else if (warp == 8) {
    if (lane == 0) {
      uint32_t ws = 0, wph = 0;
      bool wrapped = false;
      for (int work = blockIdx.x; work < numWork; work += gridDim.x) {
        const Work wk = decode_work(work, sk, nChunks);
        const int cb = wk.cb, ce = wk.ce;
        const unsigned char* src = wpack + (size_t)cb * 9 * sm.w_tile;
        for (int it = 9 * cb; it < 9 * ce; it += TPS, src += sm.w_stage) {
          if (wrapped) mbar_wait(w_empty + 8 * ws, wph ^ 1);
          mbar_arrive_expect_tx(w_full + 8 * ws, (uint32_t)sm.w_stage);
          bulk_g2s(s_base + (uint32_t)sm.w_off + ws * (uint32_t)sm.w_stage, src, (uint32_t)sm.w_stage, w_full + 8 * ws);
          if (++ws == (uint32_t)WS) { ws = 0; wph ^= 1; wrapped = true; }
        }
      }
    }
  } else {
    if (xs.in) {
      if (warp == 9 && lane == 0) {
        uint32_t as = 0, aph = 0;
        bool wrapped = false;
        for (int work = blockIdx.x; work < numWork; work += gridDim.x) {
          const Work wk = decode_work(work, sk, nChunks);
          int tx, ty, n;
          decode_tile(wk.tile, tilesX, tilesY, sk, tx, ty, n);
          const int x0 = tx * MT - dil, y0 = ty * R;
          const int gb = n * 2 * xs.in_Cg + xs.in_g0;
          for (int c = wk.cb; c < wk.ce; ++c) {
            if (wrapped) mbar_wait(a_empty + 8 * as, aph ^ 1);
            const uint32_t bar = a_full + 8 * as, dst = s_base + as * (uint32_t)sm.a_stage;
            if (dbg & 16) {
              mbar_arrive(bar);
            } else {
              mbar_arrive_expect_tx(bar, (uint32_t)sm.a_stage);
              const int g = gb + 2 * c;
              if (dil < R) {
                tma_load_4d(dst, &tmx, 0, x0, y0 - dil, g, bar);
                tma_load_4d(dst + (uint32_t)sm.a_lo, &tmx, 0, x0, y0 - dil, g + xs.in_Cg, bar);
              } else {
#pragma unroll 1
                for (int k = 0; k < 12; ++k) {
                  const int ky = k >> 2, kc = (k >> 1) & 1, pl = k & 1;
                  tma_load_4d(dst + (uint32_t)(pl * sm.a_lo + (kc * E + ky * R * PW) * 16), &tmx, 0, x0, y0 + (ky - 1) * dil,
                              g + kc + pl * xs.in_Cg, bar);
                }
              }
            }
            if (++as == (uint32_t)AS) { as = 0; aph ^= 1; wrapped = true; }
          }
        }
      }
      return;
    }
    if (dbg & 16) {
      uint32_t as = 0, aph = 0;
      bool wrapped = false;
      for (int work = blockIdx.x; work < numWork; work += gridDim.x) {
        const Work wk = decode_work(work, sk, nChunks);
        for (int c = wk.cb; c < wk.ce; ++c) {
          if (wrapped) mbar_wait(a_empty + 8 * as, aph ^ 1);
          __syncwarp();
          if (lane == 0) mbar_arrive(a_full + 8 * as);
          if (++as == (uint32_t)AS) { as = 0; aph ^= 1; wrapped = true; }
        }
      }
      return;
    }
    const int pw = warp - 9;
    const int G = (E + 31) / 32;
    const bool one_plane = Cin <= 8;
    const int nItems = one_plane ? G : 2 * G;
    const int nb = (nItems + NPROD * BATCH - 1) / (NPROD * BATCH);
    const uint32_t pw_magic = 0xFFFFFFFFu / (uint32_t)PW + 1u;
    if (one_plane) {
      for (int st = 0; st < AS; ++st)
        for (int e = pw * 32 + lane; e < E; e += NPROD * 32) {
          unsigned char* d = smem + st * sm.a_stage + (E + e) * 16;
          *reinterpret_cast<uint4*>(d) = make_uint4(0u, 0u, 0u, 0u);
          *reinterpret_cast<uint4*>(d + sm.a_lo) = make_uint4(0u, 0u, 0u, 0u);
        }
    }
    int l_work = blockIdx.x, l_c = 0, l_kb = 0, l_x0 = 0, l_y0 = 0;
    const float* l_xn = x;
    int l_ce = nChunks;
    auto set_tile = [&]() {
      const Work wk = decode_work(l_work, sk, nChunks);
      l_c = wk.cb;
      l_ce = wk.ce;
      int tx, ty, n;
      decode_tile(wk.tile, tilesX, tilesY, sk, tx, ty, n);
      l_x0 = tx * MT - (ext ? 1 : 0);
      l_y0 = ty * R - (ext ? 1 : 0);
      l_xn = x + (size_t)n * x_bs;
    };
    auto advance = [&]() {
      if (++l_kb < nb) return true;
      l_kb = 0;
      if (++l_c < l_ce) return true;
      l_work += gridDim.x;
      if (l_work >= numWork) return false;
      set_tile();
      return true;
    };
    const bool s2 = stride == 2, wide = !s2 && dil >= R;
    const int ymul = s2 ? 2 : 1, ya = s2 ? -1 : -dil, yb = wide ? dil : 0, yc = wide ? 1 : 0, yd = wide ? 0 : 1;
    const int xa = s2 ? 0 : -dil;
    const uint32_t planeu = (uint32_t)plane;
    auto load_batch = [&](float (&v)[BATCH][8]) {
      const float* xc = l_xn + (size_t)(16 * l_c) * plane;
      const int ybase = ymul * l_y0 + ya, xbase = ymul * l_x0 + xa;
#pragma unroll
      for (int b = 0; b < BATCH; ++b) {
        const int t = pw + (l_kb * BATCH + b) * NPROD;
        const int kc = one_plane ? 0 : (t & 1);
        const int e = (one_plane ? t : (t >> 1)) * 32 + lane;
        const int slot = (int)__umulhi((uint32_t)e, pw_magic), pe = e - slot * PW;
        int y = ybase + yb * (slot >> 1) + yc * (slot & 1) + yd * slot;
        const int q = (s2 && pe >= MT) ? 1 : 0;
        int xx = xbase + ymul * (pe - q * MT) - q;
        if (ext == 2) {
          y = y >= 0 ? band_map(y, H) : -1;
          xx = xx >= 0 ? band_map(xx, W) : -1;
        }
        const bool ok = t < nItems && e < E && (unsigned)y < (unsigned)H && (unsigned)xx < (unsigned)W && !(dbg & 2);
        const int c0 = 16 * l_c + 8 * kc;
        uint32_t off = (uint32_t)(8 * kc) * planeu + (ok ? (uint32_t)(y * W + xx) : 0u);
        if (c0 + 8 <= Cin) {
#pragma unroll
          for (int jj = 0; jj < 8; ++jj) {
            v[b][jj] = ok ? __ldg(xc + off) : 0.f;
            off += planeu;
          }
        } else {
#pragma unroll
          for (int jj = 0; jj < 8; ++jj) {
            v[b][jj] = (ok && c0 + jj < Cin) ? __ldg(xc + off) : 0.f;
            off += planeu;
          }
        }
      }
    };
    uint32_t as = 0, aph = 0;
    bool wrapped = false;
    auto store_batch = [&](int kb, const float (&v)[BATCH][8]) {
      if (kb == 0 && wrapped) mbar_wait(a_empty + 8 * as, aph ^ 1);
      unsigned char* a_st = smem + as * sm.a_stage;
#pragma unroll
      for (int b = 0; b < BATCH; ++b) {
        const int t = pw + (kb * BATCH + b) * NPROD;
        const int kc = one_plane ? 0 : (t & 1);
        const int e = (one_plane ? t : (t >> 1)) * 32 + lane;
        if (t < nItems && e < E) {
          uint4 hi, lo;
          split_pair(v[b][0], v[b][1], hi.x, lo.x);
          split_pair(v[b][2], v[b][3], hi.y, lo.y);
          split_pair(v[b][4], v[b][5], hi.z, lo.z);
          split_pair(v[b][6], v[b][7], hi.w, lo.w);
          unsigned char* dst = a_st + (kc * E + e) * 16;
          *reinterpret_cast<uint4*>(dst) = hi;
          *reinterpret_cast<uint4*>(dst + sm.a_lo) = lo;
        }
      }
      if (kb == nb - 1) {
        asm volatile("fence.proxy.async.shared::cta;" ::: "memory");
        __syncwarp();
        if (lane == 0) mbar_arrive(a_full + 8 * as);
        if (++as == (uint32_t)AS) { as = 0; aph ^= 1; wrapped = true; }
      }
    };
    float va[BATCH][8], vb[BATCH][8];
    set_tile();
    load_batch(va);
    int s_kb = 0;
    for (;;) {
      bool more = advance();
      if (more) load_batch(vb);
      store_batch(s_kb, va);
      if (!more) break;
      s_kb = l_kb;
      more = advance();
      if (more) load_batch(va);
      store_batch(s_kb, vb);
      if (!more) break;
      s_kb = l_kb;
    }
  }
}

long long conv3x3_wgmma_packed_bytes(int Cin, int Cout) {
  return (long long)((Cin + 15) / 16) * 9 * 64 * um::cout_pad(Cout);
}

int conv3x3_wgmma_pack(const float* weight, unsigned char* packed, int Cin, int Cout, cudaStream_t st) {
  const int CoutP = um::cout_pad(Cout), nChunks16 = (Cin + 15) / 16;
  const long long total = (long long)nChunks16 * 9 * CoutP * 8;
  long long blocks = (total + 255) / 256;
  if (blocks > 4096) blocks = 4096;
  conv3x3_pack_wgmma_kernel<<<(unsigned)blocks, 256, 0, st>>>(weight, packed, Cin, Cout, CoutP, nChunks16);
  return check_launch("conv3x3_pack_wgmma_kernel");
}

__global__ void conv3x3_wgmma_reduce_kernel(um::SplitK sk, um::SplitDev xs, int RN, const float* __restrict__ bias,
                                            float* __restrict__ out, long long out_bs, int Cout, int OH, int OW, float slope,
                                            int out_mode_arg) {
  const int out_mode = out_mode_arg & 0xff, lin_prefix = out_mode_arg >> 8;
  const long long total = (long long)RN * Cout * sk.rh * OW;
  const int F = Cout >> 2;
  for (long long i = (long long)blockIdx.x * blockDim.x + threadIdx.x; i < total; i += (long long)gridDim.x * blockDim.x) {
    float s = 0.f;
    for (int p = 0; p < sk.k; ++p) s += sk.ws[(size_t)p * (size_t)sk.part_stride + (size_t)i];
    const int x = (int)(i % OW), y = sk.y_lo + (int)((i / OW) % sk.rh), f = (int)((i / ((long long)OW * sk.rh)) % Cout);
    const int n = sk.n_lo + (int)(i / ((long long)OW * sk.rh * Cout));
    if (out_mode == 0) {
      const float b = bias ? __ldg(bias + f) : 0.f;
      const float v = leaky(s + b, f < lin_prefix ? 1.f : slope);
      if (xs.out != nullptr && f >= lin_prefix)
        sa::put_one(xs.out, xs.out_Cg, (long long)OH * OW, n, xs.out_c0 + f - lin_prefix, (long long)y * OW + x, v);
      else
        out[(size_t)n * out_bs + ((size_t)f * OH + y) * OW + x] = v;
    } else {
      const int ph = f / F, ff = f - ph * F;
      const float b = bias ? __ldg(bias + ff) : 0.f;
      out[(size_t)n * out_bs + ((size_t)ff * (2 * OH) + (2 * y + (ph >> 1))) * (2 * OW) + 2 * x + (ph & 1)] = leaky(s + b, slope);
    }
  }
}

static um::SplitK plan_split(int N, int Cin, int H, int W, int Cout, int stride, int dil, int grid_cap) {
  using namespace um;
  (void)dil;
  const int ns = cout_pad(Cout) > 128 ? 2 : 1;
  SplitK sk = {1, 0, 0, 0, 0, 0, nullptr, 0u, 0u, 3, ns};
  const int OH = (H - 1) / stride + 1, OW = (W - 1) / stride + 1, nChunks = (Cin + 15) / 16;
  const int tilesX = (OW + MT - 1) / MT, tilesY = (OH + R - 1) / R;
  const long long tiles = (long long)N * tilesX * tilesY;
  sk.from = (int)tiles;
  const int mode = tuning().conv_splitk;
  if (!mode || tiles >= (1 << 29)) return sk;
  const int sms = grid_cap > 0 && grid_cap < kNumSMs ? grid_cap : kNumSMs;
  const int kcap = mode > 1 ? mode : 32;
  if (2 * tiles * ns <= sms) {
    int k = (int)(sms / (tiles * ns));
    if (k > nChunks / 3) k = nChunks / 3;
    if (k > 8) k = 8;
    if (k > kcap) k = kcap;
    if (k >= 2) {
      sk.k = k; sk.from = 0; sk.n_lo = 0; sk.y_lo = 0; sk.rh = OH;
    }
  } else if (ns == 1 && tiles > sms) {
    const long long rounds = tiles / sms;
    long long tail = tiles - rounds * sms;
    tail = (tail + tilesX - 1) / tilesX * tilesX;
    int k = tail > 0 ? (int)(sms / tail) : 0;
    if (k > nChunks / 2) k = nChunks / 2;
    if (k > kcap) k = kcap;
    if (tail > 0 && tail <= (long long)tilesX * tilesY && rounds <= 12 && k >= 2 && nChunks >= 16 && Cout > 64) {
      sk.k = k; sk.from = (int)(tiles - tail); sk.n_lo = N - 1;
      sk.y_lo = (int)((sk.from / tilesX) % tilesY) * R;
      sk.rh = OH - sk.y_lo;
    }
  }
  if (sk.k > 1) sk.part_stride = (long long)(N - sk.n_lo) * Cout * sk.rh * OW;
  return sk;
}

long long conv3x3_wgmma_workspace_bytes(int N, int Cin, int H, int W, int Cout, int stride, int dil) {
  const um::SplitK sk = plan_split(N, Cin, H, W, Cout, stride, dil, tuning().conv_grid_cap);
  return sk.k > 1 ? sk.k * sk.part_stride * 4 : 0;
}

int conv3x3_wgmma_launch(const float* x, long long x_bs, const unsigned char* wpack, const float* bias, float* out,
                         long long out_bs, int N, int Cin, int H, int W, int Cout, int stride, int dil, int out_mode,
                         float slope, cudaStream_t st, int ext, float* ws, long long ws_bytes, const SplitIO& sio) {
  using namespace um;
  SplitDev xs = {0, 0, 0, nullptr, 0, 0};
  CUtensorMap tmx;
  memset(&tmx, 0, sizeof tmx);
  if (sio.in != nullptr) {
    if (stride != 1 || ext != 0 || sio.in_c0 % 16 != 0 || (dil >= R && dil % 2 != 0) || !aligned(sio.in, 16)) return -1;
    EncodeTiledFn fn = encode_tiled_fn();
    if (fn == nullptr) return fail(MFN_ERR_UNSUPPORTED, "cuTensorMapEncodeTiled is not available from this driver");
    const int Cg = sa::groups(sio.in_C);
    const cuuint64_t dim[4] = {8, (cuuint64_t)W, (cuuint64_t)H, (cuuint64_t)N * 2 * Cg};
    const cuuint64_t strides[3] = {16, (cuuint64_t)W * 16, (cuuint64_t)W * H * 16};
    const cuuint32_t box[4] = {8, (cuuint32_t)row_pitch(1, dil), (cuuint32_t)(dil < R ? n_slots(1, dil) : R), dil < R ? 2u : 1u};
    const cuuint32_t es[4] = {1, 1, 1, 1};
    const CUresult r = fn(&tmx, CU_TENSOR_MAP_DATA_TYPE_BFLOAT16, 4, const_cast<void*>(sio.in), dim, strides, box, es,
                          CU_TENSOR_MAP_INTERLEAVE_NONE, CU_TENSOR_MAP_SWIZZLE_NONE, CU_TENSOR_MAP_L2_PROMOTION_L2_256B,
                          CU_TENSOR_MAP_FLOAT_OOB_FILL_NONE);
    if (r != CUDA_SUCCESS) return fail(MFN_ERR_UNSUPPORTED, "cuTensorMapEncodeTiled failed (CUresult %d)", (int)r);
    xs.in = 1;
    xs.in_g0 = sio.in_c0 / 8;
    xs.in_Cg = Cg;
  }
  if (sio.out != nullptr) {
    const int lp = out_mode >> 8;
    if ((out_mode & 0xff) != 0 || ext != 0 || sio.out_c0 % 16 != 0 || (Cout - lp) % 16 != 0 || lp % 2 != 0 ||
        sio.out_c0 + Cout - lp > sio.out_C || !aligned(sio.out, 16))
      return -1;
    xs.out = static_cast<unsigned char*>(sio.out);
    xs.out_Cg = sa::groups(sio.out_C);
    xs.out_c0 = sio.out_c0;
  }
  if (Cout > 256 || (stride != 1 && !(stride == 2 && dil == 1))) return -1;
  if (ext != 0 && !((ext == 1 || ext == 2) && stride == 1 && dil == 1 && out_mode == 0)) return -1;
  if ((out_mode >> 8) != 0 && (out_mode & 0xff) != 0) return -1;
  const int CoutP = um::cout_pad(Cout), nChunks = (Cin + 15) / 16;
  const int E = n_slots(stride, dil) * row_pitch(stride, dil);
  const int as_wide = tuning().conv_as == 2 ? 2 : 3;
  const int grow = ext == 2 ? 8 : 2 * ext;
  const int OH = stride == 2 ? (H - 1) / 2 + 1 : H + grow, OW = stride == 2 ? (W - 1) / 2 + 1 : W + grow;
  const bool staged = (out_mode & 0xff) == 0 && ext == 0 &&
                      (xs.out != nullptr ? (out_mode >> 8) == 0 : OW % 4 == 0 && out_bs % 4 == 0 && aligned(out, 16)) &&
                      smem_map(E, CoutP, as_wide, STG_BYTES).WS >= 2;
  const SmemMap sm = smem_map(E, CoutP, as_wide, staged ? STG_BYTES : 0);
  if (sm.WS < 2 || E * 16 > 0x3FFF * 16) return -1;
  if ((long long)H * W >= (1LL << 27)) return -1;
  static SmemOptIn opt[8];
  {
    cudaError_t e = ensure_dyn_smem(conv3x3_wgmma_kernel<32, true, 9>, sm.total, opt[0]);
    if (e == cudaSuccess) e = ensure_dyn_smem(conv3x3_wgmma_kernel<64, true, 9>, sm.total, opt[1]);
    if (e == cudaSuccess) e = ensure_dyn_smem(conv3x3_wgmma_kernel<96, true, 3>, sm.total, opt[2]);
    if (e == cudaSuccess) e = ensure_dyn_smem(conv3x3_wgmma_kernel<128, true, 3>, sm.total, opt[3]);
    if (e == cudaSuccess) e = ensure_dyn_smem(conv3x3_wgmma_kernel<80, false, 1>, sm.total, opt[4]);
    if (e == cudaSuccess) e = ensure_dyn_smem(conv3x3_wgmma_kernel<96, false, 1>, sm.total, opt[5]);
    if (e == cudaSuccess) e = ensure_dyn_smem(conv3x3_wgmma_kernel<112, false, 1>, sm.total, opt[6]);
    if (e == cudaSuccess) e = ensure_dyn_smem(conv3x3_wgmma_kernel<128, false, 1>, sm.total, opt[7]);
    if (e != cudaSuccess) return fail((int)e, "cudaFuncSetAttribute(conv3x3_wgmma_kernel): %s", cudaGetErrorString(e));
  }
  const int tilesX = (OW + MT - 1) / MT, tilesY = (OH + R - 1) / R;
  const int ns = CoutP > 128 ? 2 : 1;
  SplitK sk = {1, 0, 0, 0, 0, 0, nullptr, 0u, 0u, 3, ns};
  if (ws != nullptr && ext == 0) {
    sk = plan_split(N, Cin, H, W, Cout, stride, dil, tuning().conv_grid_cap);
    if (sk.k > 1 && ws_bytes < sk.k * sk.part_stride * 4) sk.k = 1;
    sk.ws = ws;
  }
  const long long tiles = (long long)N * tilesX * tilesY;
  if (tiles * ns >= (1LL << 30)) return -1;
  sk.as_wide = as_wide;
  sk.stg = staged ? STG_BYTES : 0;
  if (sk.k <= 1) sk.from = (int)tiles;
  {
    const unsigned long long tp = (unsigned long long)tilesX * tilesY;
    if ((unsigned long long)tiles * tp < (1ull << 32) && tp * tilesX < (1ull << 32)) {
      sk.magic_tp = (uint32_t)(((1ull << 32) + tp - 1) / tp);
      sk.magic_tx = tilesX == 1 ? 0u : (uint32_t)(((1ull << 32) + tilesX - 1) / tilesX);
    }
    if (tp == 1) sk.magic_tp = 0;
  }
  const long long numWork = (sk.from + (tiles - sk.from) * sk.k) * ns;
  const int cap = tuning().conv_grid_cap > 0 ? tuning().conv_grid_cap : kNumSMs;
  const unsigned grid = (unsigned)(numWork < cap ? numWork : cap);
#define MFN_WGMMA_LAUNCH(NW_, FOLD_, TPS_)                                                                                   \
  conv3x3_wgmma_kernel<NW_, FOLD_, TPS_><<<grid, NTHREADS, sm.total, st>>>(x, x_bs, wpack, bias, out, out_bs, Cin, H, W, OH, \
                                                                           OW, Cout, CoutP, nChunks, slope, tilesX, tilesY,  \
                                                                           (int)numWork, stride, dil, out_mode, ext, sk, xs, \
                                                                           tmx, tuning().conv_dbg)
  const char* name = "conv3x3_wgmma_kernel<CoutP=256>";
  switch (CoutP) {
    case 16: MFN_WGMMA_LAUNCH(32, true, 9); name = "conv3x3_wgmma_kernel<CoutP=16,fold>"; break;
    case 32: MFN_WGMMA_LAUNCH(64, true, 9); name = "conv3x3_wgmma_kernel<CoutP=32,fold>"; break;
    case 48: MFN_WGMMA_LAUNCH(96, true, 3); name = "conv3x3_wgmma_kernel<CoutP=48,fold>"; break;
    case 64: MFN_WGMMA_LAUNCH(128, true, 3); name = "conv3x3_wgmma_kernel<CoutP=64,fold>"; break;
    case 80: MFN_WGMMA_LAUNCH(80, false, 1); name = "conv3x3_wgmma_kernel<CoutP=80>"; break;
    case 96: MFN_WGMMA_LAUNCH(96, false, 1); name = "conv3x3_wgmma_kernel<CoutP=96>"; break;
    case 112: MFN_WGMMA_LAUNCH(112, false, 1); name = "conv3x3_wgmma_kernel<CoutP=112>"; break;
    case 128: MFN_WGMMA_LAUNCH(128, false, 1); name = "conv3x3_wgmma_kernel<CoutP=128>"; break;
    default: MFN_WGMMA_LAUNCH(128, false, 1);
  }
#undef MFN_WGMMA_LAUNCH
  const int rc = check_launch(name);
  if (rc != 0 || sk.k <= 1) return rc;
  const long long total = sk.part_stride;
  long long blocks = (total + 255) / 256;
  if (blocks > 4 * kNumSMs) blocks = 4 * kNumSMs;
  conv3x3_wgmma_reduce_kernel<<<(unsigned)blocks, 256, 0, st>>>(sk, xs, N - sk.n_lo, bias, out, out_bs, Cout, OH, OW, slope, out_mode);
  return check_launch("conv3x3_wgmma_reduce_kernel");
}

}
```

### maskflownet_b200/csrc/mma_tiles.cuh

```cuda
#pragma once
#include <cuda_bf16.h>

#include "common.cuh"
#include "ptx.cuh"

namespace mfn {
namespace c3 {
constexpr int TW = 32, HX = 4, HWP = TW + 2 * HX;
constexpr int PXB = 64;
constexpr int NTHREADS = 256;
constexpr int WSTAGES = 3;

__host__ __device__ constexpr int cout_pad(int cout) { return cout <= 32 ? 32 : (cout <= 64 ? 64 : (cout <= 96 ? 96 : 128)); }
}

long long conv3x3_sync_packed_bytes(int Cin, int Cout);
long long conv3x3_wgmma_packed_bytes(int Cin, int Cout);
int conv3x3_wgmma_pack(const float* weight, unsigned char* packed, int Cin, int Cout, cudaStream_t st);
struct SplitIO {
  const void* in = nullptr;
  int in_C = 0, in_c0 = 0;
  void* out = nullptr;
  int out_C = 0, out_c0 = 0;
};
int conv3x3_wgmma_launch(const float* x, long long x_bs, const unsigned char* wpack, const float* bias, float* out,
                        long long out_bs, int N, int Cin, int H, int W, int Cout, int stride, int dil, int out_mode,
                        float slope, cudaStream_t st, int ext = 0, float* ws = nullptr, long long ws_bytes = 0,
                        const SplitIO& sio = SplitIO());
typedef CUresult (*EncodeTiledFn)(CUtensorMap*, CUtensorMapDataType, cuuint32_t, void*, const cuuint64_t*, const cuuint64_t*,
                                  const cuuint32_t*, const cuuint32_t*, CUtensorMapInterleave, CUtensorMapSwizzle,
                                  CUtensorMapL2promotion, CUtensorMapFloatOOBfill);
EncodeTiledFn encode_tiled_fn();
long long conv3x3_wgmma_workspace_bytes(int N, int Cin, int H, int W, int Cout, int stride, int dil);

}
```

Baseline: 728.8.

## Add narrow-image flattened tiling mode to wgmma conv3x3 kernel

Adds a NARROW template variant of the wgmma 3x3 conv for stride-1, dilation-1 layers whose output width is smaller than the tile width. It flattens several padded rows into one linear pixel tile with a single M-half, so low-resolution pyramid levels stop wasting MMA rows on out-of-bounds columns. The TMA box and loads, the output index math and tile counting are reworked to match, and the staged epilogue is turned off in this mode. It also removes the min-width tuning knob, which may send some convs that used the sync kernel through the wgmma path, and it exposes a tile-pixels query.

```diff
diff --git a/include/maskflow_b200.h b/include/maskflow_b200.h
--- a/include/maskflow_b200.h
+++ b/include/maskflow_b200.h
@@ -121,6 +121,7 @@
                                    float* out, long long out_batch_stride, int N, int Cin, int H, int W, int Cout,
                                    int stride, int dilation, int out_mode, float leaky_slope, void* stream);
 MFN_API long long mfn_conv3x3_workspace_bytes(int N, int Cin, int H, int W, int Cout, int stride, int dilation);
+MFN_API int mfn_conv3x3_tile_pixels(int N, int Cin, int H, int W, int Cout, int stride, int dilation);
 MFN_API int mfn_conv3x3_forward_ws(const float* x, long long x_batch_stride, const void* packed_weight, const float* bias,
                                    float* out, long long out_batch_stride, int N, int Cin, int H, int W, int Cout,
                                    int stride, int dilation, int out_mode, float leaky_slope, void* workspace,
diff --git a/maskflownet_b200/_lib.py b/maskflownet_b200/_lib.py
--- a/maskflownet_b200/_lib.py
+++ b/maskflownet_b200/_lib.py
@@ -49,6 +49,7 @@
     "mfn_conv3x3_forward_ws": [_f, _ll, _f, _f, _f, _ll, _i, _i, _i, _i, _i, _i, _i, _i, _fl, _f, _ll, _f],
     "mfn_conv3x3_forward_split": [_f, _i, _i, _f, _f, _f, _ll, _f, _i, _i] + [_i] * 7 + [_fl, _f, _ll, _f],
     "mfn_split_pack": [_f, _ll, _i, _i, _i, _i, _f, _i, _i, _f],
+    "mfn_conv3x3_tile_pixels": [_i] * 7,
 }
 
 
diff --git a/maskflownet_b200/csrc/api.cu b/maskflownet_b200/csrc/api.cu
--- a/maskflownet_b200/csrc/api.cu
+++ b/maskflownet_b200/csrc/api.cu
@@ -61,7 +61,7 @@
   else if (!strcmp(key, "corr_ring_th")) mfn::tuning().corr_ring_th = value;
   else if (!strcmp(key, "conv_wgmma")) mfn::tuning().conv_wgmma = value;
   else if (!strcmp(key, "conv_grid_cap")) mfn::tuning().conv_grid_cap = value;
-  else if (!strcmp(key, "conv_wgmma_min_w")) mfn::tuning().conv_wgmma_min_w = value;
+  else if (!strcmp(key, "conv_narrow")) mfn::tuning().conv_narrow = value;
   else return mfn::fail(MFN_ERR_INVALID_ARG, "mfn_set_tuning: unknown key '%s'", key);
   return MFN_OK;
 }
diff --git a/maskflownet_b200/csrc/common.cuh b/maskflownet_b200/csrc/common.cuh
--- a/maskflownet_b200/csrc/common.cuh
+++ b/maskflownet_b200/csrc/common.cuh
@@ -17,7 +17,7 @@
   int corr_disable_ring = 0;
   int conv_wgmma = 1;
   int conv_grid_cap = 0;
-  int conv_wgmma_min_w = 1;
+  int conv_narrow = 1;
   int corr_ring_th = 8;
   int corr_rb = 1;
   int warp_lin_fch = 0;
diff --git a/maskflownet_b200/csrc/conv3x3.cu b/maskflownet_b200/csrc/conv3x3.cu
--- a/maskflownet_b200/csrc/conv3x3.cu
+++ b/maskflownet_b200/csrc/conv3x3.cu
@@ -301,8 +301,13 @@
   if (N <= 0 || Cin <= 0 || H <= 0 || W <= 0 || Cout <= 0 || Cout > 256 || dilation < 1 ||
       !(stride == 1 || (stride == 2 && dilation == 1)))
     return 0;
-  if (!(tuning().conv_wgmma && W >= tuning().conv_wgmma_min_w) && Cout <= 128 && stride == 1) return 0;
+  if (!tuning().conv_wgmma && Cout <= 128 && stride == 1) return 0;
   return conv3x3_wgmma_workspace_bytes(N, Cin, H, W, Cout, stride, dilation);
+}
+
+extern "C" int mfn_conv3x3_tile_pixels(int N, int Cin, int H, int W, int Cout, int stride, int dilation) {
+  using namespace mfn;
+  return conv3x3_wgmma_tile_pixels(N, Cin, H, W, Cout, stride, dilation);
 }
 
 extern "C" int mfn_conv3x3_forward_ws(const float* x, long long x_batch_stride, const void* packed_weight,
@@ -333,7 +338,7 @@
   const unsigned char* wp = static_cast<const unsigned char*>(packed_weight);
   cudaStream_t st = as_stream(stream);
   const bool sync_ok = Cout <= 128 && stride == 1 && mode == MFN_CONV_OUT_NCHW;
-  if ((tuning().conv_wgmma && W >= tuning().conv_wgmma_min_w) || !sync_ok) {
+  if (tuning().conv_wgmma || !sync_ok) {
     const int rc = conv3x3_wgmma_launch(x, xbs, wp + conv3x3_sync_packed_bytes(Cin, Cout), bias, out, obs, N, Cin, H, W,
                                        Cout, stride, dilation, out_mode, leaky_slope, st, 0, static_cast<float*>(workspace),
                                        workspace_bytes);
diff --git a/maskflownet_b200/csrc/conv3x3_wgmma.cu b/maskflownet_b200/csrc/conv3x3_wgmma.cu
--- a/maskflownet_b200/csrc/conv3x3_wgmma.cu
+++ b/maskflownet_b200/csrc/conv3x3_wgmma.cu
@@ -1,3 +1,4 @@
+#include <cassert>
 #include <cstring>
 
 #include "mma_tiles.cuh"
@@ -22,6 +23,8 @@
 __host__ __device__ inline int tap_xoff(int kx, int stride, int dil) {
   return stride == 2 ? (kx == 1 ? 0 : (kx == 0 ? MT : MT + 1)) : kx * dil;
 }
+__host__ __device__ inline int narrow_rows(int P) { return (MT - 1) / P + 4; }
+__host__ __device__ inline int narrow_entries(int P) { return (narrow_rows(P) * P + 2 + 7) / 8 * 8; }
 __host__ __device__ inline int band_map(int v, int n) { return v < n ? v : (v == n + 2 ? 0 : (v == n + 5 ? n - 1 : -1)); }
 __host__ __device__ inline int cout_pad(int cout) { return cout <= 128 ? (cout + 15) / 16 * 16 : 256; }
 __host__ __device__ inline bool fold_hi_lo(int CoutP) { return CoutP <= 64; }
@@ -227,7 +230,7 @@
   }
 }
 
-template <int NW, bool FOLD, int TPS>
+template <int NW, bool FOLD, int TPS, bool NARROW>
 __global__ void __launch_bounds__(um::NTHREADS, 1)
     conv3x3_wgmma_kernel(const float* __restrict__ x, long long x_bs, const unsigned char* __restrict__ wpack,
                          const float* __restrict__ bias_arg, float* __restrict__ out_base, long long out_bs, int Cin, int H, int W,
@@ -236,9 +239,11 @@
                          const __grid_constant__ CUtensorMap tmx, int dbg) {
   using namespace um;
   constexpr int NCOL = FOLD ? NW / 2 : NW;
+  constexpr int MH = NARROW ? 1 : 2;
   const int out_mode_k = out_mode_arg & 0xff, lin_prefix_k = out_mode_arg >> 8;
   extern __shared__ __align__(128) unsigned char smem[];
-  const int nslots = n_slots(stride, dil), PW = row_pitch(stride, dil), E = nslots * PW;
+  const int PW = NARROW ? OW + 2 : row_pitch(stride, dil);
+  const int nslots = NARROW ? narrow_rows(PW) : n_slots(stride, dil), E = NARROW ? narrow_entries(PW) : nslots * PW;
   const SmemMap sm = smem_map(E, CoutP, sk.as_wide, sk.stg);
   const int AS = sm.AS, WS = sm.WS;
   const uint32_t s_base = smem_u32(smem);
@@ -268,7 +273,7 @@
     uint32_t a_off[9];
 #pragma unroll
     for (int tap = 0; tap < 9; ++tap)
-      a_off[tap] = (uint32_t)(slot_of(r, tap / 3, stride, dil) * PW + tap_xoff(tap % 3, stride, dil));
+      a_off[tap] = (uint32_t)(slot_of(NARROW ? 0 : r, tap / 3, stride, dil) * PW + tap_xoff(tap % 3, stride, dil));
     const uint64_t dh_a = desc_hi(a_lbo, 128u), dh_b = desc_hi(b_lbo, 128u);
     uint32_t as = 0, aph = 0, ws = 0, wph = 0;
     const uint32_t a_lo16 = (uint32_t)sm.a_lo >> 4, a_stage16 = (uint32_t)sm.a_stage >> 4, s_base16 = s_base >> 4;
@@ -282,13 +287,18 @@
       }
       rel_w = rel_a = -1;
     };
-    float acc[2][NW / 2];
+    float acc[MH][NW / 2];
     for (int work = blockIdx.x; work < numWork; work += gridDim.x) {
       const Work wk = decode_work(work, sk, nChunks);
       const int cb = wk.cb, ce = wk.ce;
       const uint32_t b_nh16 = (uint32_t)(wk.nh * NCOL);
-      fence_acc(acc[0]);
-      fence_acc(acc[1]);
+      uint32_t a_item16 = 0;
+      if constexpr (NARROW) {
+        const int v0 = (wk.tile - wk.tile / tilesX * tilesX) * MT;
+        a_item16 = (uint32_t)(v0 - v0 / PW * PW + 64 * r);
+      }
+#pragma unroll
+      for (int mh = 0; mh < MH; ++mh) fence_acc(acc[mh]);
       if (dbg & 8) {
         for (int c = cb; c < ce; ++c) {
           mbar_wait(a_full + 8 * as, aph);
@@ -306,7 +316,7 @@
       }
       for (int c = (dbg & 8) ? ce : cb; c < ce; ++c) {
         mbar_wait(a_full + 8 * as, aph);
-        const uint32_t a_st16 = s_base16 + as * a_stage16;
+        const uint32_t a_st16 = s_base16 + as * a_stage16 + a_item16;
 #pragma unroll
         for (int tap = 0; tap < 9; ++tap) {
           if (tap % TPS == 0) mbar_wait(w_full + 8 * ws, wph);
@@ -315,7 +325,7 @@
           const uint32_t sc = (tap == 0 && c == cb) ? 0u : 1u;
           wgmma_fence();
 #pragma unroll
-          for (int mh = 0; mh < 2; ++mh) {
+          for (int mh = 0; mh < MH; ++mh) {
             const uint32_t a16 = a_st16 + a_off[tap] + (uint32_t)(64 * mh);
             const uint64_t a_hi = dh_a | (uint64_t)a16, a_lo = dh_a | (uint64_t)(a16 + a_lo16);
             if constexpr (FOLD) {
@@ -339,8 +349,8 @@
         if (++as == (uint32_t)AS) { as = 0; aph ^= 1; }
       }
       wgmma_wait<0>();
-      fence_acc(acc[0]);
-      fence_acc(acc[1]);
+#pragma unroll
+      for (int mh = 0; mh < MH; ++mh) fence_acc(acc[mh]);
       release();
 
       int tx, ty, n;
@@ -356,7 +366,7 @@
       const int y = ty * R + r;
       const int F = Cout >> 2;
       const size_t oplane2 = (size_t)(2 * OH) * (2 * OW);
-      if (y < OH && !(dbg & 4) && sk.stg && !partial) {
+      if (!NARROW && y < OH && !(dbg & 4) && sk.stg && !partial) {
         constexpr int SCH = NCOL % STG_CH == 0 ? STG_CH : 16;
         float* const stg = reinterpret_cast<float*>(smem + sm.stg_off) + r * STG_CH * SPITCH;
         const int t = wq * 32 + lane;
@@ -376,7 +386,7 @@
               const float b1 = (bias != nullptr && f + 1 < Cout) ? __ldg(bias + f + 1) : 0.f;
               unsigned char* const row = sst + (2 * jj * MT + 16 * wq + (lane >> 2)) * 16 + (lane & 3) * 4;
 #pragma unroll
-              for (int mh = 0; mh < 2; ++mh)
+              for (int mh = 0; mh < MH; ++mh)
 #pragma unroll
                 for (int h = 0; h < 2; ++h) {
                   const int i = 4 * j + 2 * h;
@@ -416,7 +426,7 @@
               const float sl = f < lin_prefix ? 1.f : slope;
               float* const row = stg + (8 * jj + 2 * (lane & 3) + e) * SPITCH + 16 * wq + (lane >> 2);
 #pragma unroll
-              for (int mh = 0; mh < 2; ++mh)
+              for (int mh = 0; mh < MH; ++mh)
 #pragma unroll
                 for (int h = 0; h < 2; ++h) {
                   const int i = 4 * j + 2 * h + e;
@@ -434,13 +444,19 @@
             bulk_commit();
           }
         }
-      } else if (y < OH && !(dbg & 4)) {
-#pragma unroll
-        for (int mh = 0; mh < 2; ++mh) {
+      } else if ((NARROW || y < OH) && !(dbg & 4)) {
+#pragma unroll
+        for (int mh = 0; mh < MH; ++mh) {
 #pragma unroll
           for (int h = 0; h < 2; ++h) {
-            const int xx = tx * MT + 64 * mh + 16 * wq + (lane >> 2) + 8 * h;
-            if (xx >= OW) continue;
+            const int m = 16 * wq + (lane >> 2) + 8 * h;
+            int yy = y, xx = tx * MT + 64 * mh + m;
+            if constexpr (NARROW) {
+              const int v = tx * MT + 64 * r + m;
+              yy = v / PW;
+              xx = v - yy * PW;
+            }
+            if ((NARROW && yy >= OH) || xx >= OW) continue;
 #pragma unroll
             for (int j = 0; j < NCOL / 8; ++j) {
 #pragma unroll
@@ -455,16 +471,16 @@
                     const float b0 = bias != nullptr ? __ldg(bias + f) : 0.f, b1 = bias != nullptr ? __ldg(bias + f + 1) : 0.f;
                     float v1 = acc[mh][i + 1];
                     if constexpr (FOLD) v1 += acc[mh][i + 1 + NW / 4];
-                    sa::put_pair(xs.out, xs.out_Cg, oplane0, n, xs.out_c0 + f - lin_prefix, (size_t)y * OW + xx,
+                    sa::put_pair(xs.out, xs.out_Cg, oplane0, n, xs.out_c0 + f - lin_prefix, (size_t)yy * OW + xx,
                                  leaky(v + b0, slope), leaky(v1 + b1, slope));
                   }
                 } else if (out_mode == 0) {
                   const float t = v + (bias != nullptr ? __ldg(bias + f) : 0.f);
-                  out[(size_t)f * oplane0 + (size_t)y * OW + xx] = leaky(t, f < lin_prefix ? 1.f : slope);
+                  out[(size_t)f * oplane0 + (size_t)yy * OW + xx] = leaky(t, f < lin_prefix ? 1.f : slope);
                 } else {
                   const int ph = f / F, ff = f - ph * F;
                   const float t = v + (bias != nullptr ? __ldg(bias + ff) : 0.f);
-                  out[(size_t)ff * oplane2 + (size_t)(2 * y + (ph >> 1)) * (2 * OW) + 2 * xx + (ph & 1)] = leaky(t, slope);
+                  out[(size_t)ff * oplane2 + (size_t)(2 * yy + (ph >> 1)) * (2 * OW) + 2 * xx + (ph & 1)] = leaky(t, slope);
                 }
               }
             }
@@ -494,11 +510,12 @@
       if (warp == 9 && lane == 0) {
         uint32_t as = 0, aph = 0;
         bool wrapped = false;
+        const uint32_t a_bytes = NARROW ? (uint32_t)(4 * nslots * PW * 16) : (uint32_t)sm.a_stage;
         for (int work = blockIdx.x; work < numWork; work += gridDim.x) {
           const Work wk = decode_work(work, sk, nChunks);
           int tx, ty, n;
           decode_tile(wk.tile, tilesX, tilesY, sk, tx, ty, n);
-          const int x0 = tx * MT - dil, y0 = ty * R;
+          const int x0 = NARROW ? -1 : tx * MT - dil, y0 = NARROW ? tx * MT / PW : ty * R;
           const int gb = n * 2 * xs.in_Cg + xs.in_g0;
           for (int c = wk.cb; c < wk.ce; ++c) {
             if (wrapped) mbar_wait(a_empty + 8 * as, aph ^ 1);
@@ -506,9 +523,14 @@
             if (dbg & 16) {
               mbar_arrive(bar);
             } else {
-              mbar_arrive_expect_tx(bar, (uint32_t)sm.a_stage);
+              mbar_arrive_expect_tx(bar, a_bytes);
               const int g = gb + 2 * c;
-              if (dil < R) {
+              if (NARROW) {
+#pragma unroll
+                for (int k = 0; k < 4; ++k)
+                  tma_load_4d(dst + (uint32_t)((k >> 1) * sm.a_lo + (k & 1) * E * 16), &tmx, 0, x0, y0 - 1,
+                              g + (k & 1) + (k >> 1) * xs.in_Cg, bar);
+              } else if (dil < R) {
                 tma_load_4d(dst, &tmx, 0, x0, y0 - dil, g, bar);
                 tma_load_4d(dst + (uint32_t)sm.a_lo, &tmx, 0, x0, y0 - dil, g + xs.in_Cg, bar);
               } else {
@@ -563,8 +585,8 @@
       l_ce = wk.ce;
       int tx, ty, n;
       decode_tile(wk.tile, tilesX, tilesY, sk, tx, ty, n);
-      l_x0 = tx * MT - (ext ? 1 : 0);
-      l_y0 = ty * R - (ext ? 1 : 0);
+      l_x0 = (NARROW ? 0 : tx * MT) - (ext ? 1 : 0);
+      l_y0 = (NARROW ? tx * MT / PW : ty * R) - (ext ? 1 : 0);
       l_xn = x + (size_t)n * x_bs;
     };
     auto advance = [&]() {
@@ -738,9 +760,32 @@
   return sk;
 }
 
+static bool plan_geometry(const um::SplitK& sk, int stride, int dil, int OW) {
+  return tuning().conv_narrow && stride == 1 && dil == 1 && OW + 2 < um::MT && (sk.k <= 1 || sk.from == 0);
+}
+
 long long conv3x3_wgmma_workspace_bytes(int N, int Cin, int H, int W, int Cout, int stride, int dil) {
   const um::SplitK sk = plan_split(N, Cin, H, W, Cout, stride, dil, tuning().conv_grid_cap);
   return sk.k > 1 ? sk.k * sk.part_stride * 4 : 0;
+}
+
+int conv3x3_wgmma_tile_pixels(int N, int Cin, int H, int W, int Cout, int stride, int dil) {
+  const um::SplitK sk = plan_split(N, Cin, H, W, Cout, stride, dil, tuning().conv_grid_cap);
+  return plan_geometry(sk, stride, dil, (W - 1) / stride + 1) ? um::MT : um::R * um::MT;
+}
+
+template <bool NARROW>
+static cudaError_t wgmma_smem_opt_in(int bytes) {
+  static SmemOptIn opt[8];
+  cudaError_t e = ensure_dyn_smem(conv3x3_wgmma_kernel<32, true, 9, NARROW>, bytes, opt[0]);
+  if (e == cudaSuccess) e = ensure_dyn_smem(conv3x3_wgmma_kernel<64, true, 9, NARROW>, bytes, opt[1]);
+  if (e == cudaSuccess) e = ensure_dyn_smem(conv3x3_wgmma_kernel<96, true, 3, NARROW>, bytes, opt[2]);
+  if (e == cudaSuccess) e = ensure_dyn_smem(conv3x3_wgmma_kernel<128, true, 3, NARROW>, bytes, opt[3]);
+  if (e == cudaSuccess) e = ensure_dyn_smem(conv3x3_wgmma_kernel<80, false, 1, NARROW>, bytes, opt[4]);
+  if (e == cudaSuccess) e = ensure_dyn_smem(conv3x3_wgmma_kernel<96, false, 1, NARROW>, bytes, opt[5]);
+  if (e == cudaSuccess) e = ensure_dyn_smem(conv3x3_wgmma_kernel<112, false, 1, NARROW>, bytes, opt[6]);
+  if (e == cudaSuccess) e = ensure_dyn_smem(conv3x3_wgmma_kernel<128, false, 1, NARROW>, bytes, opt[7]);
+  return e;
 }
 
 int conv3x3_wgmma_launch(const float* x, long long x_bs, const unsigned char* wpack, const float* bias, float* out,
@@ -752,20 +797,9 @@
   memset(&tmx, 0, sizeof tmx);
   if (sio.in != nullptr) {
     if (stride != 1 || ext != 0 || sio.in_c0 % 16 != 0 || (dil >= R && dil % 2 != 0) || !aligned(sio.in, 16)) return -1;
-    EncodeTiledFn fn = encode_tiled_fn();
-    if (fn == nullptr) return fail(MFN_ERR_UNSUPPORTED, "cuTensorMapEncodeTiled is not available from this driver");
-    const int Cg = sa::groups(sio.in_C);
-    const cuuint64_t dim[4] = {8, (cuuint64_t)W, (cuuint64_t)H, (cuuint64_t)N * 2 * Cg};
-    const cuuint64_t strides[3] = {16, (cuuint64_t)W * 16, (cuuint64_t)W * H * 16};
-    const cuuint32_t box[4] = {8, (cuuint32_t)row_pitch(1, dil), (cuuint32_t)(dil < R ? n_slots(1, dil) : R), dil < R ? 2u : 1u};
-    const cuuint32_t es[4] = {1, 1, 1, 1};
-    const CUresult r = fn(&tmx, CU_TENSOR_MAP_DATA_TYPE_BFLOAT16, 4, const_cast<void*>(sio.in), dim, strides, box, es,
-                          CU_TENSOR_MAP_INTERLEAVE_NONE, CU_TENSOR_MAP_SWIZZLE_NONE, CU_TENSOR_MAP_L2_PROMOTION_L2_256B,
-                          CU_TENSOR_MAP_FLOAT_OOB_FILL_NONE);
-    if (r != CUDA_SUCCESS) return fail(MFN_ERR_UNSUPPORTED, "cuTensorMapEncodeTiled failed (CUresult %d)", (int)r);
     xs.in = 1;
     xs.in_g0 = sio.in_c0 / 8;
-    xs.in_Cg = Cg;
+    xs.in_Cg = sa::groups(sio.in_C);
   }
   if (sio.out != nullptr) {
     const int lp = out_mode >> 8;
@@ -780,33 +814,42 @@
   if (ext != 0 && !((ext == 1 || ext == 2) && stride == 1 && dil == 1 && out_mode == 0)) return -1;
   if ((out_mode >> 8) != 0 && (out_mode & 0xff) != 0) return -1;
   const int CoutP = um::cout_pad(Cout), nChunks = (Cin + 15) / 16;
-  const int E = n_slots(stride, dil) * row_pitch(stride, dil);
   const int as_wide = tuning().conv_as == 2 ? 2 : 3;
   const int grow = ext == 2 ? 8 : 2 * ext;
   const int OH = stride == 2 ? (H - 1) / 2 + 1 : H + grow, OW = stride == 2 ? (W - 1) / 2 + 1 : W + grow;
-  const bool staged = (out_mode & 0xff) == 0 && ext == 0 &&
+  const SplitK plan = plan_split(N, Cin, H, W, Cout, stride, dil, tuning().conv_grid_cap);
+  const bool narrow = plan_geometry(ext ? SplitK{} : plan, stride, dil, OW);
+  const int PW = narrow ? OW + 2 : row_pitch(stride, dil);
+  const int E = narrow ? narrow_entries(PW) : n_slots(stride, dil) * PW;
+  assert(!narrow || (PW - 1) + (MT - 1) + 2 * PW + 2 < E);
+  if (xs.in) {
+    EncodeTiledFn fn = encode_tiled_fn();
+    if (fn == nullptr) return fail(MFN_ERR_UNSUPPORTED, "cuTensorMapEncodeTiled is not available from this driver");
+    const cuuint64_t dim[4] = {8, (cuuint64_t)W, (cuuint64_t)H, (cuuint64_t)N * 2 * xs.in_Cg};
+    const cuuint64_t strides[3] = {16, (cuuint64_t)W * 16, (cuuint64_t)W * H * 16};
+    const cuuint32_t box[4] = {8, (cuuint32_t)PW, (cuuint32_t)(narrow ? narrow_rows(PW) : (dil < R ? n_slots(1, dil) : R)),
+                               !narrow && dil < R ? 2u : 1u};
+    const cuuint32_t es[4] = {1, 1, 1, 1};
+    const CUresult r = fn(&tmx, CU_TENSOR_MAP_DATA_TYPE_BFLOAT16, 4, const_cast<void*>(sio.in), dim, strides, box, es,
+                          CU_TENSOR_MAP_INTERLEAVE_NONE, CU_TENSOR_MAP_SWIZZLE_NONE, CU_TENSOR_MAP_L2_PROMOTION_L2_256B,
+                          CU_TENSOR_MAP_FLOAT_OOB_FILL_NONE);
+    if (r != CUDA_SUCCESS) return fail(MFN_ERR_UNSUPPORTED, "cuTensorMapEncodeTiled failed (CUresult %d)", (int)r);
+  }
+  const bool staged = !narrow && (out_mode & 0xff) == 0 && ext == 0 &&
                       (xs.out != nullptr ? (out_mode >> 8) == 0 : OW % 4 == 0 && out_bs % 4 == 0 && aligned(out, 16)) &&
                       smem_map(E, CoutP, as_wide, STG_BYTES).WS >= 2;
   const SmemMap sm = smem_map(E, CoutP, as_wide, staged ? STG_BYTES : 0);
   if (sm.WS < 2 || E * 16 > 0x3FFF * 16) return -1;
   if ((long long)H * W >= (1LL << 27)) return -1;
-  static SmemOptIn opt[8];
   {
-    cudaError_t e = ensure_dyn_smem(conv3x3_wgmma_kernel<32, true, 9>, sm.total, opt[0]);
-    if (e == cudaSuccess) e = ensure_dyn_smem(conv3x3_wgmma_kernel<64, true, 9>, sm.total, opt[1]);
-    if (e == cudaSuccess) e = ensure_dyn_smem(conv3x3_wgmma_kernel<96, true, 3>, sm.total, opt[2]);
-    if (e == cudaSuccess) e = ensure_dyn_smem(conv3x3_wgmma_kernel<128, true, 3>, sm.total, opt[3]);
-    if (e == cudaSuccess) e = ensure_dyn_smem(conv3x3_wgmma_kernel<80, false, 1>, sm.total, opt[4]);
-    if (e == cudaSuccess) e = ensure_dyn_smem(conv3x3_wgmma_kernel<96, false, 1>, sm.total, opt[5]);
-    if (e == cudaSuccess) e = ensure_dyn_smem(conv3x3_wgmma_kernel<112, false, 1>, sm.total, opt[6]);
-    if (e == cudaSuccess) e = ensure_dyn_smem(conv3x3_wgmma_kernel<128, false, 1>, sm.total, opt[7]);
+    const cudaError_t e = narrow ? wgmma_smem_opt_in<true>(sm.total) : wgmma_smem_opt_in<false>(sm.total);
     if (e != cudaSuccess) return fail((int)e, "cudaFuncSetAttribute(conv3x3_wgmma_kernel): %s", cudaGetErrorString(e));
   }
-  const int tilesX = (OW + MT - 1) / MT, tilesY = (OH + R - 1) / R;
+  const int tilesX = narrow ? (OH * PW + MT - 1) / MT : (OW + MT - 1) / MT, tilesY = narrow ? 1 : (OH + R - 1) / R;
   const int ns = CoutP > 128 ? 2 : 1;
   SplitK sk = {1, 0, 0, 0, 0, 0, nullptr, 0u, 0u, 3, ns};
   if (ws != nullptr && ext == 0) {
-    sk = plan_split(N, Cin, H, W, Cout, stride, dil, tuning().conv_grid_cap);
+    sk = plan;
     if (sk.k > 1 && ws_bytes < sk.k * sk.part_stride * 4) sk.k = 1;
     sk.ws = ws;
   }
@@ -826,11 +869,14 @@
   const long long numWork = (sk.from + (tiles - sk.from) * sk.k) * ns;
   const int cap = tuning().conv_grid_cap > 0 ? tuning().conv_grid_cap : kNumSMs;
   const unsigned grid = (unsigned)(numWork < cap ? numWork : cap);
-#define MFN_WGMMA_LAUNCH(NW_, FOLD_, TPS_)                                                                                   \
-  conv3x3_wgmma_kernel<NW_, FOLD_, TPS_><<<grid, NTHREADS, sm.total, st>>>(x, x_bs, wpack, bias, out, out_bs, Cin, H, W, OH, \
-                                                                           OW, Cout, CoutP, nChunks, slope, tilesX, tilesY,  \
-                                                                           (int)numWork, stride, dil, out_mode, ext, sk, xs, \
-                                                                           tmx, tuning().conv_dbg)
+#define MFN_WGMMA_ARGS                                                                                                    \
+  x, x_bs, wpack, bias, out, out_bs, Cin, H, W, OH, OW, Cout, CoutP, nChunks, slope, tilesX, tilesY, (int)numWork, stride, dil, \
+      out_mode, ext, sk, xs, tmx, tuning().conv_dbg
+#define MFN_WGMMA_LAUNCH(NW_, FOLD_, TPS_)                                                        \
+  if (narrow)                                                                                     \
+    conv3x3_wgmma_kernel<NW_, FOLD_, TPS_, true><<<grid, NTHREADS, sm.total, st>>>(MFN_WGMMA_ARGS); \
+  else                                                                                            \
+    conv3x3_wgmma_kernel<NW_, FOLD_, TPS_, false><<<grid, NTHREADS, sm.total, st>>>(MFN_WGMMA_ARGS)
   const char* name = "conv3x3_wgmma_kernel<CoutP=256>";
   switch (CoutP) {
     case 16: MFN_WGMMA_LAUNCH(32, true, 9); name = "conv3x3_wgmma_kernel<CoutP=16,fold>"; break;
@@ -844,6 +890,7 @@
     default: MFN_WGMMA_LAUNCH(128, false, 1);
   }
 #undef MFN_WGMMA_LAUNCH
+#undef MFN_WGMMA_ARGS
   const int rc = check_launch(name);
   if (rc != 0 || sk.k <= 1) return rc;
   const long long total = sk.part_stride;
diff --git a/maskflownet_b200/csrc/mma_tiles.cuh b/maskflownet_b200/csrc/mma_tiles.cuh
--- a/maskflownet_b200/csrc/mma_tiles.cuh
+++ b/maskflownet_b200/csrc/mma_tiles.cuh
@@ -32,5 +32,6 @@
                                   CUtensorMapL2promotion, CUtensorMapFloatOOBfill);
 EncodeTiledFn encode_tiled_fn();
 long long conv3x3_wgmma_workspace_bytes(int N, int Cin, int H, int W, int Cout, int stride, int dil);
+int conv3x3_wgmma_tile_pixels(int N, int Cin, int H, int W, int Cout, int stride, int dil);
 
 }
```

After: 748.0, median of 6. 1.03x the previous value.
